# ICLDisco/parsec

Hardware: NVIDIA H100
Metric: tasks/s (higher is better)
Workload: dtype i32

## Files before the change

parsec_b200/csrc/pb2_stream.cu:

```cuda
#include <cuda_runtime.h>
#include <stdio.h>
#include <stdlib.h>
#include <string.h>
#include <atomic>
#include <deque>
#include <mutex>
#include <vector>

#include "../../include/pb2_stream.h"
#include "pb2_engine_priv.hpp"
#include "pb2_worker.cuh"

namespace pb2 {

enum : uint8_t { CMD_NONE = 0, CMD_TASK = 1, CMD_TILE = 2, CMD_EDGE = 3 };
enum : uint32_t { HS_STOPPED = 0, HS_RUNNING = 1, HS_ERROR = 2 };
constexpr int32_t kEdgeEmpty = -1;
constexpr int32_t kEdgeDone = -2;

struct alignas(64) Cmd {
    uint8_t  op, body, nb_flows, flags;
    uint16_t nparts, dep_goal;
    union {
        struct { int32_t ticket; int32_t tile[PB2_MAX_FLOWS]; uint8_t access[PB2_MAX_FLOWS];
                 int32_t iparam[3]; float fparam; int32_t locals[2]; } task;
        struct { int32_t tile; int32_t state; uint32_t version; int32_t src_kind;
                 uint64_t dev_ptr; uint64_t src_ptr; uint32_t bytes; } tset;
        struct { int32_t pred, succ, node; } edge;
        uint32_t raw[12];
    } u;
    uint32_t pad;
    uint32_t stamp;
};
static_assert(sizeof(Cmd) == 64, "Cmd must be one 64-byte line");

struct alignas(32) Retire {
    uint32_t seen[PB2_MAX_FLOWS];
    uint64_t result;
    int32_t  ticket;
    uint32_t stamp;
};
static_assert(sizeof(Retire) == 32, "Retire must be 32 bytes");

struct alignas(32) TraceRec { unsigned long long t_start, t_end; uint32_t smid; int32_t ticket; uint32_t pad[2]; };

struct HostCtl {
    volatile uint32_t state;
    volatile uint32_t stop_req;
    volatile uint32_t error;
    volatile uint32_t pad;
    char pad0[48];
    volatile unsigned long long cmd_consumed;
    char pad1[56];
};

struct SCtl {
    unsigned long long cmd_head;
    unsigned long long dispatched;
    Line published;
    Line released;
    Line edges_late;
};

struct StreamDev {
    WinDev w;
    const Cmd* cmd; uint32_t cmd_mask;
    Retire* ret;   uint32_t ret_mask;
    HostCtl* hctl;
    SCtl* sctl;
    int32_t* succ_head;
    int32_t* edge_next;
    int32_t* edge_succ;
    uint16_t* nparts_rw;
    pb2_task_t* tasks_rw;
    unsigned long long idle_ns;
    TraceRec* trace;
};

__device__ __forceinline__ uint32_t ld_volatile_u32(const volatile uint32_t* p) { return *p; }
__device__ __forceinline__ void st_volatile_v4(void* p, const uint4& v) {
    asm volatile("st.volatile.global.v4.u32 [%0], {%1,%2,%3,%4};" :: "l"(p), "r"(v.x), "r"(v.y), "r"(v.z), "r"(v.w) : "memory");
}
__device__ __forceinline__ void st_volatile_v2(void* p, uint32_t a, uint32_t b) {
    asm volatile("st.volatile.global.v2.u32 [%0], {%1,%2};" :: "l"(p), "r"(a), "r"(b) : "memory");
}

__device__ __forceinline__ void push_ready(const WinDev& w, int32_t slot, int np) {
    const uint32_t first = (uint32_t)atomicAdd(&w.ctl->tail.v, (unsigned long long)np);
    for (int p = 0; p < np; ++p) st_release_gpu(&w.ring[(first + (uint32_t)p) & w.cap_mask], PB2_ENT_MAKE(slot, p));
}

__device__ __forceinline__ int32_t stream_pop(const WinDev& w) {
    const uint32_t ticket = (uint32_t)atomicAdd(&w.ctl->head.v, 1ull);
    int32_t* slot = &w.ring[ticket & w.cap_mask];
    uint32_t spins = 0;
    int32_t id;
    while ((id = ld_acquire_gpu(slot)) == kEmpty) {
        if (ld_relaxed_gpu(reinterpret_cast<const int32_t*>(&w.ctl->done.v)) != 0) return kEmpty;
        ++spins;
        __nanosleep(spins < 64 ? 32 : 256);
    }
    st_relaxed_gpu(slot, kEmpty);
    return id;
}

__device__ __forceinline__ void dispatcher_warp(const StreamDev& sd) {
    const WinDev& w = sd.w;
    const int lane = threadIdx.x & 31;
    unsigned long long head = sd.sctl->cmd_head;
    unsigned long long dispatched = sd.sctl->dispatched;
    unsigned long long last_work = globaltimer_ns();
    if (lane == 0) { sd.hctl->state = HS_RUNNING; __threadfence_system(); }
    for (;;) {
        const unsigned long long idx = head + (unsigned long long)lane;
        const Cmd* c = &sd.cmd[idx & sd.cmd_mask];
        const uint32_t want = (uint32_t)(idx / ((unsigned long long)sd.cmd_mask + 1ull)) + 1u;
        const uint32_t got = ld_volatile_u32(&c->stamp);
        const unsigned validm = __ballot_sync(0xffffffffu, got == want);
        const int n = (validm == 0xffffffffu) ? 32 : (__ffs(~validm) - 1);
        if (n == 0) {
            int leave = 0;
            if (lane == 0) {
                const unsigned long long now = globaltimer_ns();
                const unsigned long long pub = *reinterpret_cast<volatile unsigned long long*>(&sd.sctl->published.v);
                const bool quiet = (pub == dispatched);
                if (quiet && (ld_volatile_u32(&sd.hctl->stop_req) != 0 || (long long)(now - last_work) > (long long)sd.idle_ns)) {
                    sd.hctl->state = HS_STOPPED;
                    __threadfence_system();
                    if (ld_volatile_u32(&sd.cmd[head & sd.cmd_mask].stamp) == (uint32_t)(head / ((unsigned long long)sd.cmd_mask + 1ull)) + 1u) {
                        sd.hctl->state = HS_RUNNING;
                        __threadfence_system();
                    } else leave = 1;
                } else if (!quiet) {
                    const unsigned long long last = *reinterpret_cast<volatile unsigned long long*>(&w.ctl->progress_ns.v);
                    const unsigned long long ref = last > last_work ? last : last_work;
                    if ((long long)(now - ref) > (long long)w.timeout_ns) {
                        sd.hctl->error = (uint32_t)kDoneTimeout; sd.hctl->state = HS_ERROR;
                        __threadfence_system();
                        st_relaxed_gpu(reinterpret_cast<int32_t*>(&w.ctl->done.v), kDoneTimeout);
                        leave = 2;
                    }
                } else if (ld_relaxed_gpu(reinterpret_cast<const int32_t*>(&w.ctl->done.v)) == kDoneBadBody) {
                    sd.hctl->error = (uint32_t)kDoneBadBody; sd.hctl->state = HS_ERROR;
                    __threadfence_system();
                    leave = 2;
                }
            }
            leave = __shfl_sync(0xffffffffu, leave, 0);
            if (leave) {
                if (lane == 0) {
                    sd.sctl->cmd_head = head; sd.sctl->dispatched = dispatched;
                    __threadfence();
                    if (leave == 1) st_release_gpu(reinterpret_cast<int32_t*>(&w.ctl->done.v), kDoneOK);
                }
                return;
            }
            __nanosleep(200);
            continue;
        }
        __threadfence_system();
        uint4 q0 = make_uint4(0, 0, 0, 0), q1 = q0, q2 = q0, q3 = q0;
        if (lane < n) {
            const uint4* p = reinterpret_cast<const uint4*>(c);
            q0 = ld_remote(p); q1 = ld_remote(p + 1); q2 = ld_remote(p + 2); q3 = ld_remote(p + 3);
        }
        const uint8_t op = (lane < n) ? (uint8_t)(q0.x & 0xffu) : (uint8_t)CMD_NONE;
        const int np = (int)(q0.y & 0xffffu), goal = (int)(q0.y >> 16);
        int32_t ticket = -1;
        if (op == CMD_TILE) {
            const int32_t tile = (int32_t)q0.z;
            if (tile >= 0 && tile < w.ntiles) {
                pb2_tile_t t;
                t.state = (int32_t)q0.w; t.version = q1.x; t.src_kind = (int32_t)q1.y;
                t.dev_ptr = reinterpret_cast<void*>(((unsigned long long)q1.w << 32) | q1.z);
                t.src_ptr = reinterpret_cast<void*>(((unsigned long long)q2.y << 32) | q2.x);
                t.bytes = q2.z;
                w.tiles[tile] = t;
                if (w.slice_claim && t.state != PB2_TILE_VALID) {
                    for (int k = 0; k < PB2_SLICE_WORDS; ++k) w.slice_claim[(size_t)tile * PB2_SLICE_WORDS + k] = 0;
                    for (int k = 0; k <= PB2_SLICE_WORDS; ++k) w.slice_done[(size_t)tile * (PB2_SLICE_WORDS + 1) + k] = 0;
                }
            }
        } else if (op == CMD_TASK) {
            ticket = (int32_t)q0.z;
            pb2_task_t t;
            t.dep_goal = goal; t.succ_begin = 0; t.succ_count = 0; t.priority = 0;
            t.body = (uint8_t)((q0.x >> 8) & 0xffu); t.nb_flows = (uint8_t)((q0.x >> 16) & 0xffu);
            t.flags = (uint8_t)(q0.x >> 24); t.class_id = 0;
            t.tile[0] = (int32_t)q0.w; t.tile[1] = (int32_t)q1.x; t.tile[2] = (int32_t)q1.y; t.tile[3] = (int32_t)q1.z;
            t.access[0] = (uint8_t)(q1.w & 0xffu); t.access[1] = (uint8_t)((q1.w >> 8) & 0xffu);
            t.access[2] = (uint8_t)((q1.w >> 16) & 0xffu); t.access[3] = (uint8_t)(q1.w >> 24);
            t.iparam[0] = (int32_t)q2.x; t.iparam[1] = (int32_t)q2.y; t.iparam[2] = (int32_t)q2.z;
            t.fparam = __uint_as_float(q2.w);
            t.locals[0] = (int32_t)q3.x; t.locals[1] = (int32_t)q3.y;
            sd.tasks_rw[ticket] = t;
            w.dep[ticket] = goal;
            sd.succ_head[ticket] = kEdgeEmpty;
            sd.nparts_rw[ticket] = (uint16_t)np;
            w.parts_left[ticket] = np;
            w.result[ticket] = 0;
        }
        __threadfence();
        __syncwarp();
        {
            const int mine = (op == CMD_TASK && goal == 0) ? np : 0;
            int incl = mine;
            for (int o = 1; o < 32; o <<= 1) { const int v = __shfl_up_sync(0xffffffffu, incl, o); if (lane >= o) incl += v; }
            const int total = __shfl_sync(0xffffffffu, incl, 31);
            if (total) {
                unsigned long long base = 0;
                if (lane == 0) base = atomicAdd(&w.ctl->tail.v, (unsigned long long)total);
                base = __shfl_sync(0xffffffffu, base, 0);
                push_entries_warp<false>(w.ring, w.cap_mask, ticket, mine, (uint32_t)base + (uint32_t)(incl - mine));
            }
        }
        if (op == CMD_EDGE) {
            const int32_t pred = (int32_t)q0.z, succ = (int32_t)q0.w, node = (int32_t)q1.x;
            sd.edge_succ[node] = succ;
            int32_t old = ld_acquire_gpu(&sd.succ_head[pred]);
            for (;;) {
                if (old == kEdgeDone) {
                    atomicAdd(&sd.sctl->edges_late.v, 1ull);
                    if (atomicSub(&w.dep[succ], 1) == 1) push_ready(w, succ, (int)sd.nparts_rw[succ]);
                    break;
                }
                sd.edge_next[node] = old;
                __threadfence();
                const int32_t seen = atomicCAS(&sd.succ_head[pred], old, node);
                if (seen == old) break;
                old = seen;
            }
        }
        const unsigned ntask = __popc(__ballot_sync(0xffffffffu, op == CMD_TASK));
        dispatched += ntask;
        head += (unsigned long long)n;
        last_work = globaltimer_ns();
        if (lane == 0) sd.hctl->cmd_consumed = head;
    }
}

#ifndef PB2_STREAM_MINB
#define PB2_STREAM_MINB 12
#endif
__global__ void __launch_bounds__(64, PB2_STREAM_MINB)
pb2_stream_kernel(StreamDev sd) {
    const WinDev& w = sd.w;
    if (blockIdx.x == 0) {
        if (threadIdx.x < 32) dispatcher_warp(sd);
        return;
    }
    __shared__ TaskSmem s;
    __shared__ BulkSmem bulk;
    if (threadIdx.x == 0) bulk_init(bulk);
    __syncthreads();
    for (;;) {
        if (threadIdx.x == 0) {
            const int32_t e = stream_pop(w);
            if (e != kEmpty) __threadfence();
            s.entry = e;
        }
        __syncthreads();
        const int32_t entry = s.entry;
        if (entry == kEmpty) break;
        const unsigned long long t_pop = (sd.trace != nullptr && threadIdx.x == 0) ? globaltimer_ns() : 0ull;
        const int32_t id = PB2_ENT_TASK(entry);
        const int part = PB2_ENT_PART(entry);
        if (threadIdx.x < 4) reinterpret_cast<uint4*>(&s.task)[threadIdx.x] =
            __ldcg(reinterpret_cast<const uint4*>(&w.tasks[id]) + threadIdx.x);
        __syncthreads();
        const int nparts = (int)__ldcg(&w.nparts[id]);
        const unsigned long long r = run_task_part<true>(w, s, &bulk, id, part, nparts,
                                                         [&] { return run_hbm_body(s.task.body, s.args, s.red); });

        if (threadIdx.x == 0) {
            __threadfence();
            const pb2_task_t& t = s.task;
            store_result(w, t, id, part, nparts, r);
            int last = 1;
            if (nparts > 1) { last = atomicSub(&w.parts_left[id], 1) == 1; __threadfence(); }
            if (last) {
                epilog_written_flows(w, t);
                const unsigned long long ridx = atomicAdd(&w.ctl->retired.v, 1ull);
                *reinterpret_cast<volatile unsigned long long*>(&w.ctl->progress_ns.v) = globaltimer_ns();
                __threadfence();
                int32_t node = atomicExch(&sd.succ_head[id], kEdgeDone);
                while (node >= 0) {
                    const int32_t succ = __ldcg(&sd.edge_succ[node]);
                    const int32_t next = __ldcg(&sd.edge_next[node]);
                    if (atomicSub(&w.dep[succ], 1) == 1) {
                        push_ready(w, succ, (int)__ldcg(&w.nparts[succ]));
                        atomicAdd(&sd.sctl->released.v, 1ull);
                    }
                    node = next;
                }
                if (sd.trace != nullptr) {
                    TraceRec* tr = &sd.trace[ridx & sd.ret_mask];
                    tr->t_start = t_pop; tr->t_end = globaltimer_ns(); tr->smid = smid(); tr->ticket = id;
                }
                Retire* rec = &sd.ret[ridx & sd.ret_mask];
                const uint32_t gen = (uint32_t)(ridx / ((unsigned long long)sd.ret_mask + 1ull)) + 1u;
                const uint4 lo = __ldcg(reinterpret_cast<const uint4*>(&w.seen_version[(size_t)id * PB2_MAX_FLOWS]));
                const unsigned long long res = *reinterpret_cast<volatile unsigned long long*>(&w.result[id]);
                uint4 hi;
                hi.x = (uint32_t)res; hi.y = (uint32_t)(res >> 32); hi.z = (uint32_t)id;
                hi.w = (gen & 0x7fffffffu) | (r == ~0ull ? 0x80000000u : 0u);
                bool host_reads = sd.trace != nullptr;
                for (int f = 0; f < (int)t.nb_flows; ++f) host_reads |= (t.access[f] & PB2_FLOW_PUSHOUT) != 0;
                if (host_reads) __threadfence_system();
                st_volatile_v4(rec, lo);
                st_volatile_v2(&rec->result, hi.x, hi.y);
                *reinterpret_cast<volatile int32_t*>(&rec->ticket) = (int32_t)hi.z;
                st_release_sys(reinterpret_cast<int32_t*>(&rec->stamp), (int32_t)hi.w);
                __threadfence_system();
                atomicAdd(&sd.sctl->published.v, 1ull);
            }
        }
        __syncthreads();
    }
}

__global__ void pb2_stream_rearm_kernel(StreamDev sd) {
    sd.w.ctl->head.v = 0; sd.w.ctl->tail.v = 0; sd.w.ctl->done.v = 0;
    sd.w.ctl->progress_ns.v = globaltimer_ns();
}

}

using namespace pb2;

struct DryTask { pb2_task_t t; int32_t dep; std::vector<int32_t> succ; bool done; };

struct pb2_stream_s {
    pb2_engine_t* e = nullptr;
    pb2_stream_params_t p{};
    bool dry = false;
    std::string last_error;
    uint32_t slots = 0, ring_cap = 0;
    Cmd* h_cmd = nullptr; Retire* h_ret = nullptr; HostCtl* h_ctl = nullptr; TraceRec* h_trace = nullptr;
    StreamDev d{};
    std::vector<void*> dev_allocs;
    cudaStream_t kstream = nullptr;
    int nworkers = 0;
    unsigned long long cmd_written = 0;
    unsigned long long consumed_seen = 0;
    std::vector<int32_t> free_tickets, free_nodes;
    std::vector<uint64_t> cookie;
    std::vector<uint16_t> tk_parts;
    std::vector<std::vector<int32_t>> tk_nodes;
    std::vector<uint8_t> tk_live;
    alignas(64) unsigned long long ret_read = 0;
    std::vector<int32_t> freed;
    alignas(64) std::atomic<uint64_t> freed_tail{0};
    alignas(64) std::atomic<uint64_t> freed_head{0};
    alignas(64) std::atomic<uint64_t> sub_tasks{0};
    std::atomic<uint64_t> sub_entries{0};
    uint64_t ret_entries_seen = 0;
    alignas(64) std::atomic<uint64_t> ret_tasks{0};
    std::atomic<uint64_t> ret_entries{0};
    std::mutex launch_mu;
    std::mutex nodes_mu;
    std::mutex dry_mu;
    pb2_stream_stats_t st{};
    std::vector<DryTask> dry_tasks;
    std::deque<int32_t> dry_ready;
    std::vector<pb2_tile_t> dry_tiles;
    std::vector<uint32_t> tile_bytes;
};

#define STREAM_CUDA(s, call)                                                                     \
    do {                                                                                         \
        cudaError_t err__ = (call);                                                              \
        if (err__ != cudaSuccess) {                                                              \
            char buf__[512];                                                                     \
            snprintf(buf__, sizeof buf__, "%s:%d %s -> %s", __FILE__, __LINE__, #call,           \
                     cudaGetErrorString(err__));                                                 \
            (s)->last_error = buf__;                                                             \
            fprintf(stderr, "pb2: CUDA error %s\n", buf__);                                      \
            return PB2_ERR_DEVICE;                                                               \
        }                                                                                        \
    } while (0)

template <class T>
static int sdev_alloc(pb2_stream_t* s, T** out, size_t n, int fill) {
    void* ptr = nullptr;
    STREAM_CUDA(s, cudaMalloc(&ptr, (n ? n : 1) * sizeof(T)));
    STREAM_CUDA(s, cudaMemset(ptr, fill, (n ? n : 1) * sizeof(T)));
    s->dev_allocs.push_back(ptr);
    *out = reinterpret_cast<T*>(ptr);
    return PB2_SUCCESS;
}

static uint32_t round_pow2(uint32_t v, uint32_t lo, uint32_t hi) {
    uint32_t r = lo;
    while (r < v && r < hi) r <<= 1;
    return r;
}

extern "C" {

const char* pb2_stream_last_error(pb2_stream_t* s) { return s ? s->last_error.c_str() : "null stream"; }

int pb2_stream_create(pb2_engine_t* e, const pb2_stream_params_t* params, pb2_stream_t** stream) {
    if (!stream) return PB2_ERR_BAD_PARAM;
    *stream = nullptr;
    pb2_stream_params_t p{};
    if (params) p = *params;
    if (!e && !p.dry_run) return PB2_ERR_BAD_PARAM;
    if (p.cmd_slots <= 0) p.cmd_slots = 65536;
    if (p.max_tiles <= 0) p.max_tiles = 65536;
    if (p.idle_us <= 0) p.idle_us = 2000;
    if (p.timeout_ms <= 0) p.timeout_ms = 20000;
    if (p.part_bytes == 0) p.part_bytes = kDefaultPartBytes;
    pb2_stream_t* s = new pb2_stream_s();
    s->e = e; s->p = p; s->dry = p.dry_run != 0;
    s->slots = round_pow2((uint32_t)p.cmd_slots, 1024u, 1u << 21);
    s->ring_cap = s->slots * 4u;
    s->free_tickets.reserve(s->slots); s->free_nodes.reserve(s->slots);
    for (int32_t i = (int32_t)s->slots - 1; i >= 0; --i) { s->free_tickets.push_back(i); s->free_nodes.push_back(i); }
    s->tile_bytes.assign((size_t)p.max_tiles, 0);
    s->cookie.assign(s->slots, 0); s->tk_parts.assign(s->slots, 1); s->tk_nodes.resize(s->slots); s->tk_live.assign(s->slots, 0);
    s->freed.assign(s->slots, -1);
    if (s->dry) {
        s->dry_tasks.resize(s->slots);
        s->dry_tiles.resize((size_t)p.max_tiles);
        *stream = s;
        return PB2_SUCCESS;
    }
    STREAM_CUDA(s, cudaSetDevice(e->cuda_device));
    STREAM_CUDA(s, cudaHostAlloc(reinterpret_cast<void**>(&s->h_cmd), sizeof(Cmd) * s->slots, cudaHostAllocMapped | cudaHostAllocPortable));
    STREAM_CUDA(s, cudaHostAlloc(reinterpret_cast<void**>(&s->h_ret), sizeof(Retire) * s->slots, cudaHostAllocMapped | cudaHostAllocPortable));
    STREAM_CUDA(s, cudaHostAlloc(reinterpret_cast<void**>(&s->h_ctl), sizeof(HostCtl), cudaHostAllocMapped | cudaHostAllocPortable));
    memset(s->h_cmd, 0, sizeof(Cmd) * s->slots);
    memset(s->h_ret, 0, sizeof(Retire) * s->slots);
    memset((void*)s->h_ctl, 0, sizeof(HostCtl));
    StreamDev& d = s->d;
    void* alias = nullptr;
    STREAM_CUDA(s, cudaHostGetDevicePointer(&alias, s->h_cmd, 0)); d.cmd = reinterpret_cast<const Cmd*>(alias);
    STREAM_CUDA(s, cudaHostGetDevicePointer(&alias, s->h_ret, 0)); d.ret = reinterpret_cast<Retire*>(alias);
    STREAM_CUDA(s, cudaHostGetDevicePointer(&alias, (void*)s->h_ctl, 0)); d.hctl = reinterpret_cast<HostCtl*>(alias);
    d.cmd_mask = s->slots - 1; d.ret_mask = s->slots - 1;
    if (p.trace) {
        STREAM_CUDA(s, cudaHostAlloc(reinterpret_cast<void**>(&s->h_trace), sizeof(TraceRec) * s->slots, cudaHostAllocMapped | cudaHostAllocPortable));
        memset(s->h_trace, 0, sizeof(TraceRec) * s->slots);
        STREAM_CUDA(s, cudaHostGetDevicePointer(&alias, s->h_trace, 0)); d.trace = reinterpret_cast<TraceRec*>(alias);
    }
    int rc;
#define TRY(x) do { rc = (x); if (rc != PB2_SUCCESS) { pb2_stream_destroy(s); return rc; } } while (0)
    WinDev& w = d.w;
    memset(&w, 0, sizeof w);
    TRY(sdev_alloc(s, &d.tasks_rw, s->slots, 0)); w.tasks = d.tasks_rw;
    TRY(sdev_alloc(s, &w.tiles, (size_t)p.max_tiles, 0));
    TRY(sdev_alloc(s, &w.dep, s->slots, 0));
    TRY(sdev_alloc(s, &w.ring, s->ring_cap, 0xff));
    TRY(sdev_alloc(s, &w.ctl, 1, 0));
    TRY(sdev_alloc(s, &w.seen_version, (size_t)s->slots * PB2_MAX_FLOWS, 0));
    TRY(sdev_alloc(s, &w.result, s->slots, 0));
    TRY(sdev_alloc(s, &w.parts_left, s->slots, 0));
    TRY(sdev_alloc(s, &d.nparts_rw, s->slots, 0)); w.nparts = d.nparts_rw;
    TRY(sdev_alloc(s, &w.slice_claim, (size_t)p.max_tiles * PB2_SLICE_WORDS, 0));
    TRY(sdev_alloc(s, &w.slice_done, (size_t)p.max_tiles * (PB2_SLICE_WORDS + 1), 0));
    TRY(sdev_alloc(s, &d.sctl, 1, 0));
    TRY(sdev_alloc(s, &d.succ_head, s->slots, 0xff));
    TRY(sdev_alloc(s, &d.edge_next, s->slots, 0xff));
    TRY(sdev_alloc(s, &d.edge_succ, s->slots, 0xff));
#undef TRY
    w.cap_mask = s->ring_cap - 1; w.ntasks = (int32_t)s->slots; w.ntiles = p.max_tiles;
    w.stage_mode = e->params.stage_mode;
    w.part_bytes = stage_slice(e->stage_slice_bytes, p.part_bytes);
    w.timeout_ns = (unsigned long long)p.timeout_ms * 1000000ull;
    d.idle_ns = (unsigned long long)p.idle_us * 1000ull;
    STREAM_CUDA(s, cudaStreamCreateWithFlags(&s->kstream, cudaStreamNonBlocking));
    int occ = 0;
    STREAM_CUDA(s, cudaOccupancyMaxActiveBlocksPerMultiprocessor(&occ, pb2_stream_kernel, 64, 0));
    if (occ > PB2_STREAM_MINB) occ = PB2_STREAM_MINB;
    if (occ < 1) occ = 1;
    s->nworkers = e->prop.multiProcessorCount * occ;
    if (p.max_workers > 0 && p.max_workers + 1 < s->nworkers) s->nworkers = p.max_workers + 1;
    if (s->nworkers < 2) s->nworkers = 2;
    *stream = s;
    return PB2_SUCCESS;
}

int pb2_stream_destroy(pb2_stream_t* s) {
    if (!s) return PB2_ERR_BAD_PARAM;
    if (!s->dry) {
        cudaSetDevice(s->e->cuda_device);
        if (s->kstream) {
            if (s->h_ctl) s->h_ctl->stop_req = 1;
            cudaStreamSynchronize(s->kstream);
            cudaStreamDestroy(s->kstream);
        }
        for (void* p : s->dev_allocs) cudaFree(p);
        if (s->h_cmd) cudaFreeHost(s->h_cmd);
        if (s->h_ret) cudaFreeHost(s->h_ret);
        if (s->h_ctl) cudaFreeHost((void*)s->h_ctl);
        if (s->h_trace) cudaFreeHost(s->h_trace);
    }
    delete s;
    return PB2_SUCCESS;
}

static int stream_launch_if_parked(pb2_stream_t* s) {
    if (s->dry) return PB2_SUCCESS;
    std::atomic_thread_fence(std::memory_order_seq_cst);
    uint32_t st = s->h_ctl->state;
    if (st == HS_RUNNING) return PB2_SUCCESS;
    if (st == HS_ERROR) { s->last_error = "streaming kernel aborted (watchdog or unknown body)"; return PB2_ERR_DEVICE; }
    std::lock_guard<std::mutex> guard(s->launch_mu);
    st = s->h_ctl->state;
    if (st == HS_RUNNING) return PB2_SUCCESS;
    if (st == HS_ERROR) { s->last_error = "streaming kernel aborted (watchdog or unknown body)"; return PB2_ERR_DEVICE; }
    STREAM_CUDA(s, cudaSetDevice(s->e->cuda_device));
    s->h_ctl->state = HS_RUNNING;
    std::atomic_thread_fence(std::memory_order_seq_cst);
    pb2_stream_rearm_kernel<<<1, 1, 0, s->kstream>>>(s->d);
    pb2_stream_kernel<<<s->nworkers, 64, 0, s->kstream>>>(s->d);
    STREAM_CUDA(s, cudaGetLastError());
    s->st.kernel_launches++;
    return PB2_SUCCESS;
}

static int stream_cmd_slot(pb2_stream_t* s, Cmd** out) {
    if (s->cmd_written - s->consumed_seen >= (unsigned long long)s->slots) s->consumed_seen = s->h_ctl->cmd_consumed;
    if (s->cmd_written - s->consumed_seen >= (unsigned long long)s->slots) {
        int rc = stream_launch_if_parked(s);
        if (rc != PB2_SUCCESS) return rc;
        unsigned long long spins = 0;
        while (s->cmd_written - s->h_ctl->cmd_consumed >= (unsigned long long)s->slots) {
            if (s->h_ctl->state == HS_ERROR) { s->last_error = "streaming kernel aborted"; return PB2_ERR_DEVICE; }
            if ((++spins & 0xfffff) == 0 && s->h_ctl->state == HS_STOPPED) { rc = stream_launch_if_parked(s); if (rc != PB2_SUCCESS) return rc; }
        }
        s->consumed_seen = s->h_ctl->cmd_consumed;
    }
    *out = &s->h_cmd[s->cmd_written & (s->slots - 1)];
    __builtin_prefetch(&s->h_cmd[(s->cmd_written + 6) & (s->slots - 1)], 1, 3);
    return PB2_SUCCESS;
}
static void stream_cmd_publish(pb2_stream_t* s, Cmd* c) {
    const uint32_t gen = (uint32_t)(s->cmd_written / (unsigned long long)s->slots) + 1u;
    std::atomic_thread_fence(std::memory_order_release);
    *reinterpret_cast<volatile uint32_t*>(&c->stamp) = gen;
    s->cmd_written++;
}

int pb2_stream_set_tile(pb2_stream_t* s, int32_t tile, const pb2_tile_t* desc) {
    if (!s || !desc || tile < 0 || tile >= s->p.max_tiles) return PB2_ERR_BAD_PARAM;
    s->tile_bytes[(size_t)tile] = desc->bytes;
    if (s->dry) { s->dry_tiles[(size_t)tile] = *desc; return PB2_SUCCESS; }
    Cmd* c;
    int rc = stream_cmd_slot(s, &c);
    if (rc != PB2_SUCCESS) return rc;
    memset(c, 0, 60);
    c->op = CMD_TILE;
    c->u.tset.tile = tile; c->u.tset.state = desc->state; c->u.tset.version = desc->version; c->u.tset.src_kind = desc->src_kind;
    c->u.tset.dev_ptr = (uint64_t)(uintptr_t)desc->dev_ptr; c->u.tset.src_ptr = (uint64_t)(uintptr_t)desc->src_ptr;
    c->u.tset.bytes = desc->bytes;
    stream_cmd_publish(s, c);
    return PB2_SUCCESS;
}

int pb2_stream_submit(pb2_stream_t* s, const pb2_task_t* task, uint64_t cookie, int32_t* ticket) {
    if (!s || !task) return PB2_ERR_BAD_PARAM;
    if (task->nb_flows > PB2_MAX_FLOWS) { s->last_error = "task with more than PB2_MAX_FLOWS flows"; return PB2_ERR_BAD_PARAM; }
    if (task->body >= PB2_BODY_MAX || task->body == PB2_BODY_USER || task->body == PB2_BODY_GEMM_BF16) {
        s->last_error = "body cannot run in the streaming kernel"; return PB2_ERR_NOT_SUPPORTED; }
    if (task->dep_goal < 0 || task->dep_goal > 0xffff) return PB2_ERR_VALUE_OUT_OF_BOUNDS;
    for (int f = 0; f < task->nb_flows; ++f)
        if (task->tile[f] >= s->p.max_tiles) { s->last_error = "tile id out of bounds"; return PB2_ERR_VALUE_OUT_OF_BOUNDS; }
    if (s->free_tickets.empty()) {
        uint64_t h = s->freed_head.load(std::memory_order_relaxed);
        const uint64_t t = s->freed_tail.load(std::memory_order_acquire);
        for (; h != t; ++h) s->free_tickets.push_back(s->freed[h & (s->slots - 1)]);
        s->freed_head.store(h, std::memory_order_release);
        if (s->free_tickets.empty()) return PB2_ERR_OUT_OF_RESOURCE;
    }
    const uint32_t np = (uint32_t)task_parts(*task, [&](int32_t id) { return s->tile_bytes[(size_t)id]; },
                                             s->p.part_bytes, PB2_MAX_PARTS);
    {
        const uint64_t sub = s->sub_entries.load(std::memory_order_relaxed);
        if (sub - s->ret_entries_seen + np + 64 > (uint64_t)s->ring_cap / 2) {
            s->ret_entries_seen = s->ret_entries.load(std::memory_order_acquire);
            if (sub - s->ret_entries_seen + np + 64 > (uint64_t)s->ring_cap / 2) return PB2_ERR_OUT_OF_RESOURCE;
        }
    }
    const int32_t tk = s->free_tickets.back();
    if (s->dry) {
        std::lock_guard<std::mutex> guard(s->dry_mu);
        s->free_tickets.pop_back();
        s->cookie[(size_t)tk] = cookie; s->tk_parts[(size_t)tk] = (uint16_t)np; s->tk_live[(size_t)tk] = 1;
        s->sub_entries.store(s->sub_entries.load(std::memory_order_relaxed) + np, std::memory_order_relaxed);
        s->sub_tasks.store(s->sub_tasks.load(std::memory_order_relaxed) + 1, std::memory_order_release);
        if (ticket) *ticket = tk;
        DryTask& dt = s->dry_tasks[(size_t)tk];
        dt.t = *task; dt.dep = task->dep_goal; dt.succ.clear(); dt.done = false;
        if (dt.dep == 0) s->dry_ready.push_back(tk);
    } else {
        Cmd* c;
        int rc = stream_cmd_slot(s, &c);
        if (rc != PB2_SUCCESS) return rc;
        s->free_tickets.pop_back();
        s->cookie[(size_t)tk] = cookie; s->tk_parts[(size_t)tk] = (uint16_t)np; s->tk_live[(size_t)tk] = 1;
        memset(c, 0, 60);
        c->op = CMD_TASK; c->body = task->body; c->nb_flows = task->nb_flows; c->flags = task->flags;
        c->nparts = (uint16_t)np; c->dep_goal = (uint16_t)task->dep_goal;
        c->u.task.ticket = tk;
        for (int f = 0; f < PB2_MAX_FLOWS; ++f) { c->u.task.tile[f] = f < task->nb_flows ? task->tile[f] : -1; c->u.task.access[f] = task->access[f]; }
        c->u.task.iparam[0] = task->iparam[0]; c->u.task.iparam[1] = task->iparam[1]; c->u.task.iparam[2] = task->iparam[2];
        c->u.task.fparam = task->fparam; c->u.task.locals[0] = task->locals[0]; c->u.task.locals[1] = task->locals[1];
        s->sub_entries.store(s->sub_entries.load(std::memory_order_relaxed) + np, std::memory_order_relaxed);
        s->sub_tasks.store(s->sub_tasks.load(std::memory_order_relaxed) + 1, std::memory_order_release);
        if (ticket) *ticket = tk;
        stream_cmd_publish(s, c);
    }
    return PB2_SUCCESS;
}

int pb2_stream_add_edge(pb2_stream_t* s, int32_t pred, int32_t succ) {
    if (!s || pred < 0 || succ < 0 || pred >= (int32_t)s->slots || succ >= (int32_t)s->slots) return PB2_ERR_BAD_PARAM;
    if (!s->tk_live[(size_t)pred] || !s->tk_live[(size_t)succ]) { s->last_error = "edge names a ticket that is not in flight"; return PB2_ERR_BAD_PARAM; }
    s->st.edges++;
    if (s->dry) {
        std::lock_guard<std::mutex> guard(s->dry_mu);
        DryTask& p = s->dry_tasks[(size_t)pred];
        if (p.done) { if (--s->dry_tasks[(size_t)succ].dep == 0) s->dry_ready.push_back(succ); }
        else p.succ.push_back(succ);
        return PB2_SUCCESS;
    }
    Cmd* c;
    int rc = stream_cmd_slot(s, &c);
    if (rc != PB2_SUCCESS) return rc;
    int32_t node;
    {
        std::lock_guard<std::mutex> guard(s->nodes_mu);
        if (s->free_nodes.empty()) return PB2_ERR_OUT_OF_RESOURCE;
        node = s->free_nodes.back(); s->free_nodes.pop_back();
        s->tk_nodes[(size_t)pred].push_back(node);
    }
    memset(c, 0, 60);
    c->op = CMD_EDGE; c->u.edge.pred = pred; c->u.edge.succ = succ; c->u.edge.node = node;
    stream_cmd_publish(s, c);
    return PB2_SUCCESS;
}

int pb2_stream_kick(pb2_stream_t* s) {
    if (!s) return PB2_ERR_BAD_PARAM;
    if (s->dry || s->cmd_written == 0) return PB2_SUCCESS;
    return stream_launch_if_parked(s);
}

int pb2_stream_poll(pb2_stream_t* s, pb2_retire_t* out, int32_t max) {
    if (!s || (max > 0 && !out)) return PB2_ERR_BAD_PARAM;
    int n = 0;
    if (s->dry) {
        std::lock_guard<std::mutex> guard(s->dry_mu);
        while (n < max && !s->dry_ready.empty()) {
            const int32_t tk = s->dry_ready.front(); s->dry_ready.pop_front();
            DryTask& dt = s->dry_tasks[(size_t)tk];
            dt.done = true;
            pb2_retire_t& r = out[n++];
            memset(&r, 0, sizeof r);
            r.cookie = s->cookie[(size_t)tk]; r.ticket = tk; r.status = PB2_SUCCESS;
            for (int f = 0; f < dt.t.nb_flows && f < PB2_MAX_FLOWS; ++f) {
                if (dt.t.tile[f] < 0) continue;
                pb2_tile_t& tl = s->dry_tiles[(size_t)dt.t.tile[f]];
                r.seen_version[f] = tl.version;
                if (dt.t.access[f] & PB2_FLOW_ACCESS_WRITE) tl.version++;
                tl.state = PB2_TILE_VALID;
            }
            for (int32_t sc : dt.succ) if (--s->dry_tasks[(size_t)sc].dep == 0) s->dry_ready.push_back(sc);
            dt.succ.clear();
            s->tk_live[(size_t)tk] = 0;
            const uint64_t ft = s->freed_tail.load(std::memory_order_relaxed);
            s->freed[ft & (s->slots - 1)] = tk;
            s->freed_tail.store(ft + 1, std::memory_order_release);
            s->ret_entries.store(s->ret_entries.load(std::memory_order_relaxed) + s->tk_parts[(size_t)tk], std::memory_order_release);
            s->ret_tasks.store(s->ret_tasks.load(std::memory_order_relaxed) + 1, std::memory_order_release);
        }
        return n;
    }
    if (s->h_ctl->state == HS_ERROR) {
        s->last_error = s->h_ctl->error == (uint32_t)kDoneTimeout ? "streaming kernel watchdog: no task retired within timeout"
                                                                  : "streaming kernel ran a task with an unknown body id";
        return s->h_ctl->error == (uint32_t)kDoneTimeout ? PB2_ERR_DEVICE : PB2_ERR_BAD_PARAM;
    }
    if (s->h_ctl->state == HS_STOPPED && s->sub_tasks.load(std::memory_order_acquire) != s->ret_tasks.load(std::memory_order_relaxed)) {
        const Retire* nxt = &s->h_ret[s->ret_read & (s->slots - 1)];
        const uint32_t g = ((uint32_t)(s->ret_read / (unsigned long long)s->slots) + 1u) & 0x7fffffffu;
        if ((*reinterpret_cast<const volatile uint32_t*>(&nxt->stamp) & 0x7fffffffu) != g) {
            int rc = stream_launch_if_parked(s);
            if (rc != PB2_SUCCESS) return rc;
        }
    }
    while (n < max) {
        const Retire* rec = &s->h_ret[s->ret_read & (s->slots - 1)];
        __builtin_prefetch(&s->h_ret[(s->ret_read + 8) & (s->slots - 1)], 0, 3);
        const uint32_t gen = ((uint32_t)(s->ret_read / (unsigned long long)s->slots) + 1u) & 0x7fffffffu;
        const uint32_t stamp = *reinterpret_cast<const volatile uint32_t*>(&rec->stamp);
        if ((stamp & 0x7fffffffu) != gen) break;
        std::atomic_thread_fence(std::memory_order_acquire);
        const int32_t tk = *reinterpret_cast<const volatile int32_t*>(&rec->ticket);
        pb2_retire_t& r = out[n++];
        r.cookie = s->cookie[(size_t)tk]; r.result = *reinterpret_cast<const volatile uint64_t*>(&rec->result);
        for (int f = 0; f < PB2_MAX_FLOWS; ++f) r.seen_version[f] = *reinterpret_cast<const volatile uint32_t*>(&rec->seen[f]);
        r.ticket = tk; r.status = (stamp & 0x80000000u) ? PB2_ERR_BAD_PARAM : PB2_SUCCESS;
        if (s->h_trace) {
            const volatile TraceRec* tr = &s->h_trace[s->ret_read & (s->slots - 1)];
            r.t_start_ns = tr->t_start; r.t_end_ns = tr->t_end; r.smid = tr->smid; r.pad = 0;
        } else { r.t_start_ns = 0; r.t_end_ns = 0; r.smid = 0; r.pad = 0; }
        if (!s->tk_nodes[(size_t)tk].empty()) {
            std::lock_guard<std::mutex> guard(s->nodes_mu);
            for (int32_t nd : s->tk_nodes[(size_t)tk]) s->free_nodes.push_back(nd);
            s->tk_nodes[(size_t)tk].clear();
        }
        s->tk_live[(size_t)tk] = 0;
        const uint64_t ft = s->freed_tail.load(std::memory_order_relaxed);
        s->freed[ft & (s->slots - 1)] = tk;
        s->freed_tail.store(ft + 1, std::memory_order_release);
        s->ret_entries.store(s->ret_entries.load(std::memory_order_relaxed) + s->tk_parts[(size_t)tk], std::memory_order_release);
        s->ret_tasks.store(s->ret_tasks.load(std::memory_order_relaxed) + 1, std::memory_order_release);
        s->ret_read++;
    }
    return n;
}

int pb2_stream_quiesce(pb2_stream_t* s) {
    if (!s) return PB2_ERR_BAD_PARAM;
    if (s->dry) return PB2_SUCCESS;
    STREAM_CUDA(s, cudaSetDevice(s->e->cuda_device));
    if (s->cmd_written != s->h_ctl->cmd_consumed) { int rc = stream_launch_if_parked(s); if (rc != PB2_SUCCESS) return rc; }
    s->h_ctl->stop_req = 1;
    std::atomic_thread_fence(std::memory_order_seq_cst);
    STREAM_CUDA(s, cudaStreamSynchronize(s->kstream));
    s->h_ctl->stop_req = 0;
    if (s->h_ctl->state == HS_ERROR) { s->last_error = "streaming kernel aborted"; return PB2_ERR_DEVICE; }
    if (s->cmd_written != s->h_ctl->cmd_consumed) return pb2_stream_quiesce(s);
    return PB2_SUCCESS;
}

int pb2_stream_inflight(pb2_stream_t* s) { return s ? (int)(s->sub_tasks.load() - s->ret_tasks.load()) : 0; }

int pb2_stream_stats(pb2_stream_t* s, pb2_stream_stats_t* out) {
    if (!s || !out) return PB2_ERR_BAD_PARAM;
    if (!s->dry) {
        STREAM_CUDA(s, cudaSetDevice(s->e->cuda_device));
        Ctl c; SCtl sc;
        cudaStream_t aux = s->e->up_stream;
        STREAM_CUDA(s, cudaMemcpyAsync(&c, s->d.w.ctl, sizeof c, cudaMemcpyDeviceToHost, aux));
        STREAM_CUDA(s, cudaMemcpyAsync(&sc, s->d.sctl, sizeof sc, cudaMemcpyDeviceToHost, aux));
        STREAM_CUDA(s, cudaStreamSynchronize(aux));
        s->st.bytes_h2d = c.bytes_h2d.v; s->st.bytes_d2d = c.bytes_d2d.v; s->st.bytes_d2h = c.bytes_d2h.v;
        s->st.stage_ins = c.stage_ins.v; s->st.body_errors = c.body_errors.v;
        s->st.edges_late = sc.edges_late.v; s->st.released_on_device = sc.released.v;
    }
    s->st.submitted = s->sub_tasks.load(); s->st.retired = s->ret_tasks.load();
    *out = s->st;
    return PB2_SUCCESS;
}

}
```

parsec_b200/mca/b200/device_b200_module.c:

```c
#include "parsec/parsec_config.h"
#include "parsec/parsec_internal.h"
#include "parsec/sys/atomic.h"
#include "parsec/utils/mca_param.h"
#include "parsec/utils/debug.h"
#include "parsec/utils/zone_malloc.h"
#include "parsec/constants.h"
#include "parsec/data_internal.h"
#include "parsec/scheduling.h"
#include "parsec/execution_stream.h"
#include "parsec/mca/device/device.h"
#include "parsec/mca/device/device_gpu.h"
#include "parsec/mca/device/b200/device_b200.h"
#include "parsec/mca/device/b200/device_b200_internal.h"

#include "pb2_engine.h"
#include "pb2_stream.h"

#include <cuda_runtime_api.h>
#include <stddef.h>
#include <stdlib.h>
#include <string.h>
#include <stdio.h>
#include <limits.h>
#include <time.h>
static inline uint64_t b200_now_ns(void) { struct timespec ts; clock_gettime(CLOCK_MONOTONIC, &ts); return (uint64_t)ts.tv_sec * 1000000000ull + (uint64_t)ts.tv_nsec; }
#include <x86intrin.h>
#define B200_TSC() __rdtsc()

#include <nvtx3/nvToolsExt.h>
static nvtxDomainHandle_t b200_nvtx_domain = NULL;
static inline void b200_nvtx_attr(nvtxEventAttributes_t *a, const char *name)
{
    memset(a, 0, sizeof *a);
    a->version = NVTX_VERSION; a->size = NVTX_EVENT_ATTRIB_STRUCT_SIZE;
    a->messageType = NVTX_MESSAGE_TYPE_ASCII; a->message.ascii = name;
}
static inline void b200_nvtx_push(const char *name)
{
    if( parsec_b200_nvtx ) { nvtxEventAttributes_t a; b200_nvtx_attr(&a, name); (void)nvtxDomainRangePushEx(b200_nvtx_domain, &a); }
}
static inline void b200_nvtx_pop(void)
{
    if( parsec_b200_nvtx ) (void)nvtxDomainRangePop(b200_nvtx_domain);
}
static inline void b200_nvtx_mark(const char *name)
{
    if( parsec_b200_nvtx ) { nvtxEventAttributes_t a; b200_nvtx_attr(&a, name); nvtxDomainMarkEx(b200_nvtx_domain, &a); }
}

typedef struct b200_lock_s {
    volatile uint32_t next;    char pad0[60];
    volatile uint32_t serving; char pad1[60];
} b200_lock_t;
static inline void b200_lock(b200_lock_t *l)
{
    const uint32_t t = __atomic_fetch_add(&l->next, 1, __ATOMIC_RELAXED);
    while( __atomic_load_n(&l->serving, __ATOMIC_ACQUIRE) != t ) _mm_pause();
}
static inline void b200_unlock(b200_lock_t *l)
{
    __atomic_store_n(&l->serving, l->serving + 1, __ATOMIC_RELEASE);
}

enum {
    BT_NEW = 0,
    BT_STAGED,
    BT_DMA_IN,
    BT_INFLIGHT,
    BT_LANE,
    BT_DMA_OUT
};

typedef struct b200_task_s {
    parsec_list_item_t   item;
    parsec_gpu_task_t   *gpu_task;
    int32_t              state;
    int32_t              ticket;
    int32_t              body;
    int32_t              prepared;
    int32_t              cmd_built;
    int32_t              recorded;
    int32_t              has_complete_stage;
    uint32_t             dma_out_mask;
    uint64_t             result;
    uint64_t             cold_bytes;
    struct parsec_device_b200_module_s *dev;
    int32_t              is_kernel;
    int32_t              defer_tiles;
    int32_t              ntdesc;
    pb2_task_t           cmd __attribute__((aligned(64)));
    parsec_task_t        proxy __attribute__((aligned(64)));
    int32_t              nb_args;
    int32_t              arg_flow[PB2_MAX_FLOWS];
    int32_t              iparam[3];
    float                fparam;
    uint32_t             peer_src_mask;
    parsec_data_copy_t  *peer_src[MAX_PARAM_COUNT];
    int32_t              custom_stage;
    cudaEvent_t          ev;
    int32_t              ev_dev;
    struct b200_task_s  *next_free;
    struct b200_task_s  *next_done;
    struct { int32_t tile; pb2_tile_t desc; } tdesc[MAX_PARAM_COUNT];
} b200_task_t;

typedef struct b200_host_range_s { char *base; size_t len; char *alias; int lazy; } b200_host_range_t;

typedef struct b200_trace_ev_s {
    char     name[24];
    int32_t  locals[2];
    int32_t  body, smid;
    uint64_t t_start_ns, t_end_ns, cold_bytes;
} b200_trace_ev_t;
#define B200_LINE __attribute__((aligned(64)))
typedef struct parsec_device_b200_module_s {
    parsec_device_cuda_module_t super;
    pb2_engine_t        *engine;
    pb2_stream_t        *stream;
    int                  dry_run;
    char                *slab_base;
    uint8_t             *tile_described;
    b200_task_t * volatile *inbox_ring;
    cudaStream_t         dma_stream;
    parsec_cuda_exec_stream_t *lane;
    uint64_t             first_entry_ns, first_task_ns, last_done_ns;
    volatile int64_t     inbox_tail B200_LINE;
    volatile int32_t     owed B200_LINE;
    volatile int32_t     callers_inside B200_LINE;
    volatile int32_t     max_callers_inside;
    volatile int64_t     epilogs_done B200_LINE;
    b200_lock_t          lru_lock B200_LINE;
    b200_lock_t          alloc_lock B200_LINE;
    volatile int32_t     handed_back B200_LINE;
    volatile int32_t     starter_active B200_LINE;
    volatile int32_t     fatal;
    volatile int32_t     memory_pressure;
    struct b200_task_s * volatile lane_done;
    volatile int32_t     retry_stalled B200_LINE;
    volatile int64_t     cold_inflight B200_LINE;
    volatile int64_t     inbox_head B200_LINE;
    parsec_list_t        stalled B200_LINE;
    parsec_list_t        settled;
    parsec_list_t        cold_q;
    int32_t              nb_cold;
    parsec_list_t        waiting_event;
    int32_t              nb_settled;
    int32_t              nb_stalled;
    int32_t              again_window;
    int32_t              lane_pending;
    uint64_t             n_engine, n_lane, n_settled_by_caller;
    uint64_t             tsc_start[4];
    uint64_t             tsc_s[3];
    parsec_list_t        waiting_out B200_LINE;
    parsec_task_t       *completion_ring;
    b200_task_t         *batch_head;
    int32_t              batch_len;
    int32_t              completed_now;
    int32_t              blocked_spins;
    int32_t              complete_inline;
    int64_t              epilogs_started;
    uint64_t             tsc[8];
    struct b200_trace_ev_s *trace_ev;
    size_t               trace_n, trace_cap;
    pb2_retire_t         retbuf[256];
    parsec_b200_stats_t  st B200_LINE;
} parsec_device_b200_module_t;

static b200_host_range_t *b200_ranges = NULL;
static int b200_nb_ranges = 0, b200_cap_ranges = 0;
static parsec_atomic_lock_t b200_ranges_lock = PARSEC_ATOMIC_UNLOCKED;

static int  parsec_b200_submit_is_engine(parsec_advance_task_function_t fn);
static void parsec_b200_submit_set_engine(parsec_advance_task_function_t fn);

#define B200_DEV(gpu)   ((parsec_device_b200_module_t*)(gpu))
#define B200_BT(gt)     ((b200_task_t*)(uintptr_t)(gt)->last_data_check_epoch)

#define B200_CUDA(call, what, onerr)                                                              \
    do { cudaError_t e__ = (call); if( cudaSuccess != e__ ) {                                     \
        parsec_warning("device_b200: %s: %s", (what), cudaGetErrorString(e__)); onerr; } } while(0)

int parsec_b200_is_b200_device(const parsec_device_module_t *device)
{
    return (NULL != device) && (device->component == &parsec_device_b200_component);
}

int parsec_b200_device_count(void)
{
    int n = 0;
    if( cudaSuccess != cudaGetDeviceCount(&n) ) { (void)cudaGetLastError(); return 0; }
    return n;
}

static char *b200_device_visible(const void *host_ptr, size_t len)
{
    char *res = NULL;
    parsec_atomic_lock(&b200_ranges_lock);
    for( int i = 0; i < b200_nb_ranges; i++ ) {
        const b200_host_range_t *r = &b200_ranges[i];
        if( (const char*)host_ptr >= r->base && (const char*)host_ptr + len <= r->base + r->len ) {
            res = r->alias + ((const char*)host_ptr - r->base);
            break;
        }
    }
    parsec_atomic_unlock(&b200_ranges_lock);
    return res;
}

#define B200_INBOX_SLOTS (1 << 16)
#define B200_TL_CACHE    8192
#define B200_FLAG_WRITER ((parsec_data_flag_t)1 << 4)
static __thread b200_task_t *b200_tl_free = NULL;
static __thread int          b200_tl_nfree = 0;
static __thread b200_task_t *b200_tl_recording = NULL;

static parsec_hook_return_t b200_epilog_hook(parsec_execution_stream_t *es, parsec_task_t *task);
static const __parsec_chore_t b200_completion_chores[] = {
    { .type = PARSEC_DEV_CPU, .evaluate = NULL, .hook = b200_epilog_hook, .dyld = NULL, .dyld_fn = NULL },
    { .type = PARSEC_DEV_NONE, .evaluate = NULL, .hook = NULL, .dyld = NULL, .dyld_fn = NULL },
};
static const parsec_task_class_t b200_completion_tc = {
    .name = "b200 completion", .flags = 0, .task_class_id = 0, .nb_flows = 0, .nb_parameters = 0, .nb_locals = 0,
    .incarnations = b200_completion_chores,
};

static b200_task_t *b200_bt_new(parsec_device_b200_module_t *dev, parsec_gpu_task_t *gpu_task)
{
    b200_task_t *bt = b200_tl_free;
    if( NULL != bt ) { b200_tl_free = bt->next_free; b200_tl_nfree--; }
    else {
        if( 0 != posix_memalign((void**)&bt, 64, sizeof(b200_task_t)) ) abort();
        memset(bt, 0, sizeof(b200_task_t));
        PARSEC_OBJ_CONSTRUCT(&bt->item, parsec_list_item_t);
        PARSEC_OBJ_CONSTRUCT(&bt->proxy, parsec_task_t);
        bt->proxy.task_class = &b200_completion_tc;
        bt->proxy.priority = INT32_MAX;
        bt->proxy.status = PARSEC_TASK_STATUS_HOOK;
        bt->proxy.chore_mask = 1;
        bt->proxy.selected_chore = 0;
        bt->proxy.selected_device = parsec_mca_device_get(0);
        bt->proxy.load = 0;
        bt->proxy.repo_entry = NULL;
        bt->ev_dev = -1;
    }
    PARSEC_LIST_ITEM_SINGLETON(&bt->item);
    bt->dev = dev;
    bt->gpu_task = gpu_task; bt->state = BT_NEW; bt->ticket = -1; bt->body = -1; bt->nb_args = 0;
    bt->peer_src_mask = 0; bt->dma_out_mask = 0; bt->result = 0; bt->custom_stage = 0; bt->cold_bytes = 0;
    bt->recorded = 0; bt->has_complete_stage = 0; bt->prepared = 0; bt->cmd_built = 0; bt->defer_tiles = 0; bt->ntdesc = 0;
    bt->is_kernel = (NULL == gpu_task) || (PARSEC_GPU_TASK_TYPE_KERNEL == gpu_task->task_type);
    if( NULL != gpu_task ) gpu_task->last_data_check_epoch = (uint64_t)(uintptr_t)bt;
    return bt;
}

static void b200_bt_free(b200_task_t *bt)
{
    bt->gpu_task = NULL;
    if( b200_tl_nfree < B200_TL_CACHE ) { bt->next_free = b200_tl_free; b200_tl_free = bt; b200_tl_nfree++; return; }
    if( bt->ev_dev >= 0 ) (void)cudaEventDestroy(bt->ev);
    free(bt);
}

static inline void b200_cuda_here(parsec_device_b200_module_t *dev)
{
    if( !dev->dry_run ) B200_CUDA(cudaSetDevice(dev->super.cuda_index), "cudaSetDevice", {});
}

static cudaEvent_t b200_bt_event(parsec_device_b200_module_t *dev, b200_task_t *bt)
{
    if( bt->ev_dev != (int32_t)dev->super.cuda_index ) {
        if( bt->ev_dev >= 0 ) (void)cudaEventDestroy(bt->ev);
        bt->ev_dev = -1;
        b200_cuda_here(dev);
        B200_CUDA(cudaEventCreateWithFlags(&bt->ev, cudaEventDisableTiming), "cudaEventCreate", { return bt->ev; });
        bt->ev_dev = (int32_t)dev->super.cuda_index;
    }
    return bt->ev;
}

static inline void b200_lru_put(parsec_device_b200_module_t *dev, parsec_list_t *list, parsec_data_copy_t *copy)
{
    b200_lock(&dev->lru_lock);
    copy->flags &= (parsec_data_flag_t)~B200_FLAG_WRITER;
    parsec_list_item_ring_chop((parsec_list_item_t*)copy); PARSEC_LIST_ITEM_SINGLETON(copy);
    parsec_list_nolock_push_back(list, (parsec_list_item_t*)copy);
    b200_unlock(&dev->lru_lock);
}
static inline void b200_lru_take(parsec_device_b200_module_t *dev, parsec_data_copy_t *copy, int for_writer)
{
    b200_lock(&dev->lru_lock);
    if( for_writer ) copy->flags |= B200_FLAG_WRITER;
    parsec_list_item_ring_chop((parsec_list_item_t*)copy); PARSEC_LIST_ITEM_SINGLETON(copy);
    b200_unlock(&dev->lru_lock);
}
static inline void b200_lru_touch(parsec_device_b200_module_t *dev, parsec_data_copy_t *copy)
{
    b200_lock(&dev->lru_lock);
    if( !(copy->flags & B200_FLAG_WRITER) ) {
        parsec_list_t *l = (PARSEC_DATA_COHERENCY_OWNED == copy->coherency_state) ? &dev->super.super.gpu_mem_owned_lru
                                                                                  : &dev->super.super.gpu_mem_lru;
        parsec_list_item_ring_chop((parsec_list_item_t*)copy); PARSEC_LIST_ITEM_SINGLETON(copy);
        parsec_list_nolock_push_back(l, (parsec_list_item_t*)copy);
    }
    b200_unlock(&dev->lru_lock);
}

#define B200_PF(p) __builtin_prefetch((const void*)(p), 0, 3)
#define B200_PFW(p) __builtin_prefetch((const void*)(p), 1, 3)
static inline void b200_pf1(const b200_task_t *bt)
{
    const char *g = (const char*)bt->gpu_task;
    if( NULL != g ) { B200_PF(g); B200_PF(g + 64); B200_PF(g + 128); }
}
static inline void b200_pf2(const b200_task_t *bt)
{
    const parsec_gpu_task_t *g = bt->gpu_task;
    if( NULL == g || NULL == g->ec ) return;
    const parsec_task_t *t = g->ec;
    B200_PF(t); B200_PF((const char*)t + 64);
    B200_PF(&t->data[0]); B200_PF((const char*)&t->data[0] + 64);
    B200_PF(g->flow_info);
}
static inline void b200_pf3(const b200_task_t *bt)
{
    const parsec_gpu_task_t *g = bt->gpu_task;
    if( NULL == g || NULL == g->ec ) return;
    const uint32_t n = g->nb_flows < 4 ? g->nb_flows : 4;
    for( uint32_t i = 0; i < n; i++ ) {
        if( NULL != g->ec->data[i].data_in ) B200_PF(g->ec->data[i].data_in);
        if( NULL != g->ec->data[i].data_out ) B200_PF(g->ec->data[i].data_out);
    }
}
static inline void b200_pf4(const b200_task_t *bt)
{
    const parsec_gpu_task_t *g = bt->gpu_task;
    if( NULL == g || NULL == g->ec ) return;
    const uint32_t n = g->nb_flows < 4 ? g->nb_flows : 4;
    for( uint32_t i = 0; i < n; i++ ) {
        const parsec_data_copy_t *c = (NULL != g->ec->data[i].data_in) ? g->ec->data[i].data_in : g->ec->data[i].data_out;
        if( NULL != c && NULL != c->original ) { B200_PF(c->original); B200_PF((const char*)c->original + 64); }
    }
}

static inline int32_t b200_tile_of(const parsec_device_b200_module_t *dev, const parsec_data_copy_t *gpu_copy)
{
    return (int32_t)(((char*)gpu_copy->device_private - dev->slab_base) / (ptrdiff_t)dev->super.super.mem_block_size);
}

static int b200_copy_acquire_reader(parsec_data_copy_t *copy)
{
    int32_t r = copy->readers;
    while( r >= 0 ) {
        if( parsec_atomic_cas_int32(&copy->readers, r, r + 1) ) return 1;
        r = copy->readers;
    }
    return 0;
}

static void b200_release_copy_memory(parsec_device_b200_module_t *dev, parsec_data_copy_t *copy)
{
    parsec_data_t *original = copy->original;
    if( NULL != original ) {
        parsec_atomic_lock(&original->lock);
        const int survives = original->super.obj_reference_count != 1;
        parsec_data_copy_detach(original, copy, dev->super.super.super.device_index);
        parsec_atomic_wmb();
        if( survives ) parsec_atomic_unlock(&original->lock);
    }
    if( NULL != dev->tile_described ) dev->tile_described[b200_tile_of(dev, copy)] = 0;
    zone_free(dev->super.super.memory, copy->device_private);
    copy->device_private = NULL;
    PARSEC_OBJ_RELEASE(copy);
    dev->super.super.super.nb_evictions++;
    dev->st.evictions++;
}

static int b200_write_back_some(parsec_device_b200_module_t *dev, int how_many)
{
    parsec_list_item_t *it, *next;
    parsec_data_copy_t *moved[64];
    int done = 0;
    if( how_many > 64 ) how_many = 64;
    b200_lock(&dev->lru_lock);
    for( it = PARSEC_LIST_ITERATOR_FIRST(&dev->super.super.gpu_mem_owned_lru);
         it != PARSEC_LIST_ITERATOR_END(&dev->super.super.gpu_mem_owned_lru) && done < how_many; it = next ) {
        parsec_data_copy_t *copy = (parsec_data_copy_t*)it;
        next = PARSEC_LIST_ITERATOR_NEXT(it);
        if( 0 != copy->readers || (copy->flags & B200_FLAG_WRITER) ) continue;
        parsec_data_copy_t *cpu = copy->original->device_copies[0];
        if( NULL == cpu || (!dev->dry_run && NULL == cpu->device_private) ) continue;
        parsec_list_nolock_remove(&dev->super.super.gpu_mem_owned_lru, it);
        PARSEC_LIST_ITEM_SINGLETON(it);
        moved[done++] = copy;
    }
    b200_unlock(&dev->lru_lock);
    if( 0 == done ) return 0;
    if( !dev->dry_run ) {
        b200_cuda_here(dev);
        for( int i = 0; i < done; i++ ) {
            parsec_data_copy_t *copy = moved[i], *cpu = copy->original->device_copies[0];
            B200_CUDA(cudaMemcpyAsync(cpu->device_private, copy->device_private, copy->original->span, cudaMemcpyDeviceToHost, dev->dma_stream),
                      "write-back cudaMemcpyAsync", { moved[i] = NULL; b200_lru_put(dev, &dev->super.super.gpu_mem_owned_lru, copy); continue; });
            (void)parsec_atomic_fetch_add_int64((volatile int64_t*)&dev->super.super.super.data_out_to_host, (int64_t)copy->original->span);
            dev->st.bytes_d2h_dma += copy->original->span;
        }
        B200_CUDA(cudaStreamSynchronize(dev->dma_stream), "write-back synchronize", {});
    }
    int n = 0;
    for( int i = 0; i < done; i++ ) {
        parsec_data_copy_t *copy = moved[i];
        if( NULL == copy ) continue;
        parsec_data_copy_t *cpu = copy->original->device_copies[0];
        parsec_atomic_lock(&copy->original->lock);
        if( cpu->version < copy->version ) cpu->version = copy->version;
        cpu->coherency_state = PARSEC_DATA_COHERENCY_SHARED;
        copy->coherency_state = PARSEC_DATA_COHERENCY_SHARED;
        if( copy->original->owner_device == (int8_t)dev->super.super.super.device_index ) copy->original->owner_device = 0;
        parsec_atomic_unlock(&copy->original->lock);
        b200_lru_put(dev, &dev->super.super.gpu_mem_lru, copy);
        dev->st.w2r_copies++;
        n++;
    }
    return n;
}

static int b200_evict_one(parsec_device_b200_module_t *dev, const parsec_gpu_task_t *for_task)
{
    for( int pass = 0; pass < 2; pass++ ) {
        parsec_list_item_t *it, *next;
        parsec_data_copy_t *victim = NULL;
        b200_lock(&dev->lru_lock);
        for( it = PARSEC_LIST_ITERATOR_FIRST(&dev->super.super.gpu_mem_lru);
             it != PARSEC_LIST_ITERATOR_END(&dev->super.super.gpu_mem_lru); it = next ) {
            parsec_data_copy_t *copy = (parsec_data_copy_t*)it;
            next = PARSEC_LIST_ITERATOR_NEXT(it);
            if( PARSEC_DATA_STATUS_UNDER_TRANSFER == copy->data_transfer_status || (copy->flags & B200_FLAG_WRITER) ) continue;
            if( copy->super.super.obj_reference_count > 1 ) continue;
            if( NULL != for_task ) {
                int mine = 0;
                for( uint32_t f = 0; f < for_task->nb_flows; f++ )
                    mine |= (for_task->ec->data[f].data_out == copy) || (for_task->ec->data[f].data_in == copy);
                if( mine ) continue;
            }
            if( !parsec_atomic_cas_int32(&copy->readers, 0, INT_MIN / 2) ) continue;
            parsec_data_copy_t *cpu = (NULL != copy->original) ? copy->original->device_copies[0] : NULL;
            if( NULL != copy->original && (NULL == cpu || cpu->version < copy->version) &&
                copy->original->owner_device == (int8_t)dev->super.super.super.device_index ) {
                copy->readers = 0;
                continue;
            }
            parsec_list_nolock_remove(&dev->super.super.gpu_mem_lru, it);
            PARSEC_LIST_ITEM_SINGLETON(it);
            victim = copy;
            break;
        }
        b200_unlock(&dev->lru_lock);
        if( NULL != victim ) {
            victim->readers = 0;
            b200_release_copy_memory(dev, victim);
            return 1;
        }
        if( 0 == b200_write_back_some(dev, 16) ) break;
    }
    return 0;
}

static int b200_reserve(parsec_device_b200_module_t *dev, b200_task_t *bt)
{
    parsec_gpu_task_t *gpu_task = bt->gpu_task;
    parsec_task_t *this_task = gpu_task->ec;
    const uint8_t my = dev->super.super.super.device_index;
    parsec_data_copy_t *fresh[MAX_PARAM_COUNT];
    int nfresh = 0;

    for( uint32_t i = 0; i < gpu_task->nb_flows; i++ ) {
        const parsec_flow_t *flow = gpu_task->flow_info[i].flow;
        if( PARSEC_FLOW_ACCESS_NONE == (PARSEC_FLOW_ACCESS_MASK & flow->flow_flags) ) { gpu_task->flow_info[i].flow_span = 0; continue; }
        parsec_data_copy_t *in = this_task->data[i].data_in;
        if( NULL == in ) continue;
        if( in->device_index == my ) { this_task->data[i].data_out = in; continue; }
        parsec_data_t *master = in->original;
        parsec_atomic_lock(&master->lock);
        parsec_data_copy_t *gpu_elem = PARSEC_DATA_GET_COPY(master, my);
        parsec_atomic_unlock(&master->lock);
        if( NULL == gpu_elem ) {
            void *ptr;
            while( NULL == (ptr = zone_malloc(dev->super.super.memory, gpu_task->flow_info[i].flow_span)) ) {
                dev->memory_pressure = 1;
                if( !b200_evict_one(dev, gpu_task) ) {
                    for( int k = 0; k < nfresh; k++ ) {
                        b200_lru_take(dev, fresh[k], 0);
                        b200_release_copy_memory(dev, fresh[k]);
                        dev->super.super.super.nb_evictions--; dev->st.evictions--;
                    }
                    for( uint32_t k = 0; k < gpu_task->nb_flows; k++ )
                        if( NULL != this_task->data[k].data_in && this_task->data[k].data_in->device_index != my ) this_task->data[k].data_out = NULL;
                    return PARSEC_HOOK_RETURN_AGAIN;
                }
            }
            gpu_elem = PARSEC_OBJ_NEW(parsec_data_copy_t);
            gpu_elem->flags = PARSEC_DATA_FLAG_PARSEC_OWNED | PARSEC_DATA_FLAG_PARSEC_MANAGED;
            gpu_elem->device_private = ptr;
            gpu_elem->arena_chunk = (parsec_arena_chunk_t*)dev->super.super.memory;
            gpu_elem->coherency_state = PARSEC_DATA_COHERENCY_INVALID;
            gpu_elem->version = 0;
            gpu_elem->dtt = in->dtt;
            parsec_atomic_lock(&master->lock);
            parsec_data_copy_attach(master, gpu_elem, my);
            parsec_atomic_unlock(&master->lock);
            b200_lru_put(dev, &dev->super.super.gpu_mem_lru, gpu_elem);
            fresh[nfresh++] = gpu_elem;
        }
        this_task->data[i].data_out = gpu_elem;
    }
    return PARSEC_HOOK_RETURN_DONE;
}

static int b200_needs_memory(const parsec_device_b200_module_t *dev, const parsec_gpu_task_t *gpu_task)
{
    const uint8_t my = dev->super.super.super.device_index;
    for( uint32_t i = 0; i < gpu_task->nb_flows; i++ ) {
        const parsec_flow_t *flow = gpu_task->flow_info[i].flow;
        if( PARSEC_FLOW_ACCESS_NONE == (PARSEC_FLOW_ACCESS_MASK & flow->flow_flags) ) continue;
        const parsec_data_copy_t *in = gpu_task->ec->data[i].data_in;
        if( NULL == in || in->device_index == my ) continue;
        if( NULL == PARSEC_DATA_GET_COPY(in->original, my) ) return 1;
    }
    return 0;
}

static int b200_emit_tile(parsec_device_b200_module_t *dev, b200_task_t *bt, int32_t tid, const pb2_tile_t *tile)
{
    if( !bt->defer_tiles ) return (PB2_SUCCESS == pb2_stream_set_tile(dev->stream, tid, tile)) ? 0 : -1;
    if( bt->ntdesc >= MAX_PARAM_COUNT ) return -1;
    bt->tdesc[bt->ntdesc].tile = tid; bt->tdesc[bt->ntdesc].desc = *tile; bt->ntdesc++;
    return 0;
}

static int b200_stage_in(parsec_device_b200_module_t *dev, b200_task_t *bt, int mode)
{
    const int for_lane = (0 != mode);
    parsec_gpu_task_t *gpu_task = bt->gpu_task;
    parsec_task_t *this_task = gpu_task->ec;
    parsec_device_module_t *mod = &dev->super.super.super;
    const uint8_t my = mod->device_index;
    int used_dma = 0;
    uint32_t pre_acquired = 0;

    for( uint32_t i = 0; i < gpu_task->nb_flows; i++ ) {
        const parsec_flow_t *flow = gpu_task->flow_info[i].flow;
        parsec_data_copy_t *in = this_task->data[i].data_in;
        if( NULL == in || NULL == this_task->data[i].data_out || in == this_task->data[i].data_out ) continue;
        if( !(PARSEC_FLOW_ACCESS_READ & flow->flow_flags) || !parsec_mca_device_is_gpu(in->device_index) ) continue;
        if( b200_copy_acquire_reader(in) ) { pre_acquired |= (1u << i); continue; }
        for( uint32_t k = 0; k < i; k++ )
            if( pre_acquired & (1u << k) ) (void)parsec_atomic_fetch_dec_int32(&this_task->data[k].data_in->readers);
        return PARSEC_HOOK_RETURN_AGAIN;
    }

    for( uint32_t i = 0; i < gpu_task->nb_flows; i++ ) {
        const parsec_flow_t *flow = gpu_task->flow_info[i].flow;
        const uint8_t type = (uint8_t)(flow->flow_flags & PARSEC_FLOW_ACCESS_MASK);
        if( PARSEC_FLOW_ACCESS_NONE == type ) continue;
        parsec_data_copy_t *in = this_task->data[i].data_in, *out = this_task->data[i].data_out;
        if( NULL == in || NULL == out ) continue;
        parsec_data_t *original = in->original;
        const size_t span = gpu_task->flow_info[i].flow_span;
        gpu_task->flow_info[i].source = NULL;

        if( in == out ) {
            if( PARSEC_FLOW_ACCESS_WRITE & type ) {
                out->version++;
                b200_lru_take(dev, out, 1);
                parsec_atomic_lock(&original->lock);
                original->owner_device = my; out->coherency_state = PARSEC_DATA_COHERENCY_OWNED;
                parsec_atomic_unlock(&original->lock);
            }
            if( PARSEC_FLOW_ACCESS_READ & type ) (void)parsec_atomic_fetch_inc_int32(&out->readers);
            if( !for_lane && !dev->tile_described[b200_tile_of(dev, out)] ) {
                pb2_tile_t tile;
                memset(&tile, 0, sizeof tile);
                tile.dev_ptr = out->device_private; tile.bytes = (uint32_t)span; tile.state = PB2_TILE_VALID;
                tile.version = (PARSEC_FLOW_ACCESS_WRITE & type) ? out->version - 1 : out->version;
                if( NULL != original->device_copies[0] && NULL != original->device_copies[0]->device_private )
                    tile.src_ptr = b200_device_visible(original->device_copies[0]->device_private, span);
                if( 0 != b200_emit_tile(dev, bt, b200_tile_of(dev, out), &tile) ) return PARSEC_HOOK_RETURN_ERROR;
                dev->tile_described[b200_tile_of(dev, out)] = 1;
            }
            continue;
        }

        parsec_atomic_lock(&original->lock);
        if( PARSEC_FLOW_ACCESS_WRITE & type ) {
            b200_lru_take(dev, out, 1);
        }
        parsec_data_copy_t *src = in;
        int src_acquired = 0, src_detour = 0;
        if( (PARSEC_FLOW_ACCESS_READ & type) ) {
            if( parsec_mca_device_is_gpu(in->device_index) ) {
                src_acquired = (pre_acquired >> i) & 1;
                src_detour = !(dev->super.super.peer_access_mask & (1 << in->device_index));
            } else if( !(PARSEC_FLOW_ACCESS_WRITE & type) ) {
                for( uint32_t t = 1; t < parsec_nb_devices; t++ ) {
                    parsec_data_copy_t *cand = original->device_copies[t];
                    if( t == my || NULL == cand || !(dev->super.super.peer_access_mask & (1 << t)) ) continue;
                    if( cand->version != in->version || PARSEC_DATA_COHERENCY_INVALID == cand->coherency_state ||
                        PARSEC_DATA_STATUS_UNDER_TRANSFER == cand->data_transfer_status ) continue;
                    if( b200_copy_acquire_reader(cand) ) { src = cand; src_acquired = 1; break; }
                }
            }
        }
        if( NULL == src ) { parsec_atomic_unlock(&original->lock); return PARSEC_HOOK_RETURN_ERROR; }

        int transfer_from = parsec_data_start_transfer_ownership_to_copy(original, my, type);
        if( -1 != transfer_from && out->version == src->version && PARSEC_DATA_STATUS_COMPLETE_TRANSFER == out->data_transfer_status ) transfer_from = -1;
        if( NULL == src->device_private ) transfer_from = -1;
        if( (NULL == this_task->data[i].source_repo_entry) && (NULL == original->dc) && (0 == in->version) ) transfer_from = -1;
        if( PARSEC_DATA_STATUS_UNDER_TRANSFER == out->data_transfer_status ) transfer_from = -1;
        mod->required_data_in += original->span;

        pb2_tile_t tile;
        memset(&tile, 0, sizeof tile);
        tile.dev_ptr = out->device_private;
        tile.bytes = (uint32_t)span;
        tile.state = PB2_TILE_VALID;
        tile.src_kind = parsec_mca_device_is_gpu(src->device_index) ? PB2_SRC_PEER : PB2_SRC_HOST;
        char *home = NULL;
        if( NULL != original->device_copies[0] && NULL != original->device_copies[0]->device_private )
            home = b200_device_visible(original->device_copies[0]->device_private, span);
        tile.src_ptr = home;

        if( -1 == transfer_from ) {
            if( src_acquired ) { (void)parsec_atomic_fetch_dec_int32(&src->readers); src_acquired = 0; }
            if( PARSEC_DATA_STATUS_UNDER_TRANSFER != out->data_transfer_status ) {
                out->data_transfer_status = PARSEC_DATA_STATUS_COMPLETE_TRANSFER;
                parsec_data_end_transfer_ownership_to_copy(original, my, type);
            }
            if( PARSEC_FLOW_ACCESS_WRITE & type ) out->version = src->version + 1;
        } else {
            char *visible = (PB2_SRC_PEER == tile.src_kind) ? (char*)src->device_private
                                                            : b200_device_visible(src->device_private, span);
            mod->data_in_from_device[src->device_index] += span;
            mod->nb_data_faults += span;
            bt->cold_bytes += span;
            if( PB2_SRC_PEER == tile.src_kind ) { if( src_detour ) dev->st.peer_detours++; else dev->st.peer_pulls++; }
            if( NULL != visible && !src_detour && !for_lane && !dev->dry_run ) {
                tile.state = PB2_TILE_INVALID;
                tile.src_ptr = visible;
                out->data_transfer_status = PARSEC_DATA_STATUS_UNDER_TRANSFER;
                if( PB2_SRC_PEER == tile.src_kind ) dev->st.bytes_d2d_kernel += span; else dev->st.bytes_h2d_kernel += span;
            } else if( 2 == mode ) {
                out->data_transfer_status = PARSEC_DATA_STATUS_UNDER_TRANSFER;
                used_dma = 1;
            } else if( !dev->dry_run ) {
                b200_cuda_here(dev);
                B200_CUDA(cudaMemcpyAsync(out->device_private, src->device_private, span,
                                          PB2_SRC_PEER == tile.src_kind ? cudaMemcpyDeviceToDevice : cudaMemcpyHostToDevice,
                                          for_lane ? dev->lane->cuda_stream : dev->dma_stream),
                          "stage-in cudaMemcpyAsync", { parsec_atomic_unlock(&original->lock); return PARSEC_HOOK_RETURN_ERROR; });
                out->data_transfer_status = PARSEC_DATA_STATUS_UNDER_TRANSFER;
                dev->st.bytes_h2d_dma += span;
                used_dma = 1;
            } else {
                out->data_transfer_status = PARSEC_DATA_STATUS_UNDER_TRANSFER;
            }
            out->version = (PARSEC_FLOW_ACCESS_WRITE & type) ? src->version + 1 : src->version;
            gpu_task->flow_info[i].source = src;
            if( src_acquired ) { bt->peer_src_mask |= (1u << i); bt->peer_src[i] = src; }
            if( PB2_SRC_PEER == tile.src_kind && PB2_TILE_INVALID == tile.state && NULL != home && (gpu_task->pushout & (1 << i)) ) {
            }
        }
        tile.version = (PARSEC_FLOW_ACCESS_WRITE & type) ? out->version - 1 : out->version;
        if( !for_lane ) {
            const int32_t tid = b200_tile_of(dev, out);
            if( -1 != transfer_from || !dev->tile_described[tid] ) {
                if( 0 != b200_emit_tile(dev, bt, tid, &tile) ) { parsec_atomic_unlock(&original->lock); return PARSEC_HOOK_RETURN_ERROR; }
                dev->tile_described[tid] = 1;
            }
        }
        parsec_atomic_unlock(&original->lock);
    }
    return used_dma;
}

int parsec_b200_task_body(parsec_device_gpu_module_t *gpu_device, parsec_gpu_task_t *gpu_task,
                          parsec_gpu_exec_stream_t *gpu_stream,
                          int body, int nb_args, const int *flow_index, const int32_t *iparam, float fparam)
{
    if( NULL == gpu_device || NULL == gpu_task || nb_args < 0 || nb_args > PB2_MAX_FLOWS || body < 0 || body >= PB2_BODY_MAX )
        return PARSEC_HOOK_RETURN_ERROR;
    for( int a = 0; a < nb_args; a++ )
        if( flow_index[a] < 0 || (uint32_t)flow_index[a] >= gpu_task->nb_flows ) return PARSEC_HOOK_RETURN_ERROR;
    if( parsec_b200_is_b200_device(&gpu_device->super) ) {
        b200_task_t *bt = b200_tl_recording;
        if( NULL == bt || bt->gpu_task != gpu_task ) return PARSEC_HOOK_RETURN_ERROR;
        bt->body = body; bt->nb_args = nb_args;
        for( int a = 0; a < nb_args; a++ ) bt->arg_flow[a] = flow_index[a];
        bt->iparam[0] = iparam ? iparam[0] : 0; bt->iparam[1] = iparam ? iparam[1] : 0; bt->iparam[2] = iparam ? iparam[2] : 0;
        bt->fparam = fparam;
        return PARSEC_HOOK_RETURN_DONE;
    }
    {
        void *ptrs[PB2_MAX_FLOWS] = {NULL, NULL, NULL, NULL};
        uint64_t bytes[PB2_MAX_FLOWS] = {0, 0, 0, 0};
        int32_t ip[3] = { iparam ? iparam[0] : 0, iparam ? iparam[1] : 0, iparam ? iparam[2] : 0 };
        for( int a = 0; a < nb_args; a++ ) {
            ptrs[a] = gpu_task->ec->data[flow_index[a]].data_out->device_private;
            bytes[a] = gpu_task->flow_info[flow_index[a]].flow_span;
        }
        parsec_cuda_exec_stream_t *cs = (parsec_cuda_exec_stream_t*)gpu_stream;
        return (PB2_SUCCESS == pb2_body_launch((void*)cs->cuda_stream, body, nb_args, ptrs, bytes, ip, fparam))
               ? PARSEC_HOOK_RETURN_DONE : PARSEC_HOOK_RETURN_ERROR;
    }
}

uint64_t parsec_b200_task_result(const parsec_gpu_task_t *gpu_task)
{
    const b200_task_t *bt = (const b200_task_t*)(uintptr_t)gpu_task->last_data_check_epoch;
    return (NULL != bt) ? bt->result : 0;
}

static inline void b200_stat_add(uint64_t *counter, uint64_t v)
{
    (void)parsec_atomic_fetch_add_int64((volatile int64_t*)counter, (int64_t)v);
}

static int b200_epilog_flows(parsec_device_b200_module_t *dev, b200_task_t *bt, parsec_data_copy_t **held)
{
    parsec_gpu_task_t *gpu_task = bt->gpu_task;
    parsec_task_t *this_task = gpu_task->ec;
    parsec_device_module_t *mod = &dev->super.super.super;
    int nheld = 0;

    for( uint32_t i = 0; i < gpu_task->nb_flows; i++ ) {
        const parsec_flow_t *flow = gpu_task->flow_info[i].flow;
        const uint8_t type = (uint8_t)(flow->flow_flags & PARSEC_FLOW_ACCESS_MASK);
        if( PARSEC_FLOW_ACCESS_NONE == type || NULL == this_task->data[i].data_in ) continue;
        parsec_data_copy_t *gpu_copy = this_task->data[i].data_out;
        if( NULL == gpu_copy ) continue;
        parsec_data_t *original = gpu_copy->original;
        const int locked = (PARSEC_FLOW_ACCESS_WRITE & type) || PARSEC_DATA_STATUS_UNDER_TRANSFER == gpu_copy->data_transfer_status;
        if( locked ) parsec_atomic_lock(&original->lock);
        if( PARSEC_DATA_STATUS_UNDER_TRANSFER == gpu_copy->data_transfer_status ) {
            gpu_copy->data_transfer_status = PARSEC_DATA_STATUS_COMPLETE_TRANSFER;
            parsec_data_end_transfer_ownership_to_copy(original, mod->device_index, type);
        }
        if( bt->peer_src_mask & (1u << i) ) (void)parsec_atomic_fetch_dec_int32(&bt->peer_src[i]->readers);
        if( !(PARSEC_FLOW_ACCESS_READ & type) ) (void)parsec_atomic_fetch_inc_int32(&gpu_copy->readers);
        held[nheld++] = gpu_copy;
        if( PARSEC_FLOW_ACCESS_WRITE & type ) {
            b200_stat_add(&mod->required_data_out, gpu_task->flow_info[i].flow_span);
            if( gpu_task->pushout & (1 << i) ) {
                parsec_data_copy_t *cpu_copy = original->device_copies[0];
                if( NULL != cpu_copy ) {
                    cpu_copy->version = gpu_copy->version;
                    cpu_copy->coherency_state = PARSEC_DATA_COHERENCY_SHARED;
                    gpu_copy->coherency_state = PARSEC_DATA_COHERENCY_SHARED;
                    cpu_copy->data_transfer_status = PARSEC_DATA_STATUS_COMPLETE_TRANSFER;
                    b200_stat_add(&mod->data_out_to_host, gpu_task->flow_info[i].flow_span);
                    if( 0 == (parsec_mpi_allow_gpu_memory_communications & PARSEC_RUNTIME_SEND_GPU_MEMORY) )
                        this_task->data[i].data_out = cpu_copy;
                }
                b200_lru_put(dev, &dev->super.super.gpu_mem_lru, gpu_copy);
            } else {
                gpu_copy->coherency_state = PARSEC_DATA_COHERENCY_OWNED;
                b200_lru_put(dev, &dev->super.super.gpu_mem_owned_lru, gpu_copy);
            }
        } else if( dev->memory_pressure && 1 == gpu_copy->readers && 0 != (gpu_copy->flags & PARSEC_DATA_FLAG_PARSEC_OWNED) ) {
            b200_lru_touch(dev, gpu_copy);
        }
        if( locked ) parsec_atomic_unlock(&original->lock);
    }
    return nheld;
}

static parsec_hook_return_t b200_epilog_hook(parsec_execution_stream_t *es, parsec_task_t *task)
{
    b200_task_t *bt = (b200_task_t*)((char*)task - offsetof(b200_task_t, proxy));
    parsec_device_b200_module_t *dev = bt->dev;
    int64_t n = 0;
    b200_nvtx_push("b200 epilog batch");
    while( NULL != bt ) {
        b200_task_t *next = bt->next_done;
        parsec_gpu_task_t *gpu_task = bt->gpu_task;
        parsec_data_copy_t *held[MAX_PARAM_COUNT];
        if( NULL != next ) { B200_PF(next); B200_PF(next->gpu_task); }
        const int nheld = b200_epilog_flows(dev, bt, held);
        (void)__parsec_complete_execution(es, gpu_task->ec);
        for( int i = 0; i < nheld; i++ ) (void)parsec_atomic_fetch_dec_int32(&held[i]->readers);
        gpu_task->last_data_check_epoch = 0;
        gpu_task->release_device_task(gpu_task);
        b200_bt_free(bt);
        bt = next;
        n++;
    }
    if( dev->nb_stalled > 0 && !dev->retry_stalled ) dev->retry_stalled = 1;
    parsec_atomic_wmb();
    (void)parsec_atomic_fetch_add_int64(&dev->epilogs_done, n);
    b200_nvtx_pop();
    return PARSEC_HOOK_RETURN_ASYNC;
}

#define B200_EPILOG_BATCH 4
static inline void b200_close_batch(parsec_device_b200_module_t *dev)
{
    b200_task_t *bt = dev->batch_head;
    if( NULL == bt ) return;
    dev->batch_head = NULL; dev->batch_len = 0;
    PARSEC_LIST_ITEM_SINGLETON(&bt->proxy);
    if( NULL == dev->completion_ring ) dev->completion_ring = &bt->proxy;
    else parsec_list_item_ring_push((parsec_list_item_t*)dev->completion_ring, (parsec_list_item_t*)&bt->proxy);
}

static void b200_complete(parsec_device_b200_module_t *dev, parsec_execution_stream_t *es, b200_task_t *bt)
{
    dev->super.super.super.executed_tasks++;
    dev->completed_now++;
    if( parsec_b200_parallel_completion && !bt->has_complete_stage && !dev->complete_inline ) {
        dev->epilogs_started++;
        bt->next_done = dev->batch_head; dev->batch_head = bt;
        if( ++dev->batch_len >= B200_EPILOG_BATCH ) b200_close_batch(dev);
        return;
    }
    parsec_gpu_task_t *gpu_task = bt->gpu_task;
    parsec_data_copy_t *held[MAX_PARAM_COUNT];
    const int nheld = b200_epilog_flows(dev, bt, held);
    if( NULL != gpu_task->complete_stage ) {
        parsec_gpu_task_t *gt = gpu_task;
        (void)gpu_task->complete_stage(&dev->super.super, &gt, &dev->lane->super);
    }
    __parsec_complete_execution(es, gpu_task->ec);
    for( int i = 0; i < nheld; i++ ) (void)parsec_atomic_fetch_dec_int32(&held[i]->readers);
    gpu_task->last_data_check_epoch = 0;
    gpu_task->release_device_task(gpu_task);
    b200_bt_free(bt);
}

static int b200_dma_pushout(parsec_device_b200_module_t *dev, b200_task_t *bt)
{
    parsec_gpu_task_t *gpu_task = bt->gpu_task;
    int n = 0;
    if( dev->dry_run ) return 0;
    b200_cuda_here(dev);
    if( NULL != gpu_task->stage_out && gpu_task->stage_out != parsec_default_gpu_stage_out ) {
        if( PARSEC_SUCCESS != gpu_task->stage_out(gpu_task, bt->dma_out_mask, &dev->lane->super) ) return 0;
        B200_CUDA(cudaEventRecord(b200_bt_event(dev, bt), dev->lane->cuda_stream), "cudaEventRecord", {});
        return 1;
    }
    for( uint32_t i = 0; i < gpu_task->nb_flows; i++ ) {
        if( !(bt->dma_out_mask & (1u << i)) ) continue;
        parsec_data_copy_t *gpu_copy = gpu_task->ec->data[i].data_out;
        parsec_data_copy_t *cpu_copy = gpu_copy->original->device_copies[0];
        if( NULL == cpu_copy || NULL == cpu_copy->device_private ) continue;
        B200_CUDA(cudaMemcpyAsync(cpu_copy->device_private, gpu_copy->device_private, gpu_task->flow_info[i].flow_span,
                                  cudaMemcpyDeviceToHost, dev->dma_stream), "pushout cudaMemcpyAsync", { continue; });
        dev->st.bytes_d2h_dma += gpu_task->flow_info[i].flow_span;
        n++;
    }
    if( n ) B200_CUDA(cudaEventRecord(b200_bt_event(dev, bt), dev->dma_stream), "cudaEventRecord", {});
    return n;
}

static void b200_build_cmd(parsec_device_b200_module_t *dev, b200_task_t *bt)
{
    parsec_gpu_task_t *gpu_task = bt->gpu_task;
    pb2_task_t *t = &bt->cmd;
    memset(t, 0, sizeof *t);
    t->body = (uint8_t)bt->body; t->nb_flows = (uint8_t)bt->nb_args;
    for( int a = 0; a < PB2_MAX_FLOWS; a++ ) t->tile[a] = -1;
    for( int a = 0; a < bt->nb_args; a++ ) {
        const int f = bt->arg_flow[a];
        const parsec_flow_t *flow = gpu_task->flow_info[f].flow;
        parsec_data_copy_t *out = gpu_task->ec->data[f].data_out;
        t->tile[a] = b200_tile_of(dev, out);
        t->access[a] = (uint8_t)(flow->flow_flags & PARSEC_FLOW_ACCESS_MASK);
        if( (gpu_task->pushout & (1 << f)) && (PARSEC_FLOW_ACCESS_WRITE & flow->flow_flags) ) {
            parsec_data_copy_t *cpu = out->original->device_copies[0];
            if( !bt->custom_stage && NULL != cpu && NULL != cpu->device_private &&
                NULL != b200_device_visible(cpu->device_private, gpu_task->flow_info[f].flow_span) && !(bt->peer_src_mask & (1u << f)) )
                t->access[a] |= PB2_FLOW_PUSHOUT;
            else bt->dma_out_mask |= (1u << f);
        }
    }
    for( uint32_t f = 0; f < gpu_task->nb_flows; f++ ) {
        int named = 0;
        for( int a = 0; a < bt->nb_args; a++ ) named |= (bt->arg_flow[a] == (int)f);
        if( !named && (gpu_task->pushout & (1 << f)) && (PARSEC_FLOW_ACCESS_WRITE & gpu_task->flow_info[f].flow->flow_flags) &&
            NULL != gpu_task->ec->data[f].data_out ) bt->dma_out_mask |= (1u << f);
    }
    t->iparam[0] = bt->iparam[0]; t->iparam[1] = bt->iparam[1]; t->iparam[2] = bt->iparam[2]; t->fparam = bt->fparam;
    t->locals[0] = gpu_task->ec->locals[0].value; t->locals[1] = gpu_task->ec->locals[1].value;
    bt->cmd_built = 1;
}

static int b200_push_engine(parsec_device_b200_module_t *dev, b200_task_t *bt)
{
    if( !bt->cmd_built ) b200_build_cmd(dev, bt);
    const int32_t state_before = bt->state;
    bt->state = BT_INFLIGHT;
    int rc = pb2_stream_submit(dev->stream, &bt->cmd, (uint64_t)(uintptr_t)bt, &bt->ticket);
    if( PB2_SUCCESS != rc ) {
        bt->state = state_before;
        if( PB2_ERR_OUT_OF_RESOURCE == rc ) return PARSEC_HOOK_RETURN_AGAIN;
        parsec_warning("device_b200: submit failed: %s", pb2_stream_last_error(dev->stream));
        return PARSEC_HOOK_RETURN_ERROR;
    }
    dev->n_engine++;
    return PARSEC_HOOK_RETURN_DONE;
}

static int b200_prepare_resident(parsec_device_b200_module_t *dev, b200_task_t *bt)
{
    parsec_gpu_task_t *gpu_task = bt->gpu_task;
    parsec_task_t *this_task = gpu_task->ec;
    const uint8_t my = dev->super.super.super.device_index;
    if( NULL == dev->tile_described ) return 0;
    for( uint32_t i = 0; i < gpu_task->nb_flows; i++ ) {
        const parsec_flow_t *flow = gpu_task->flow_info[i].flow;
        if( PARSEC_FLOW_ACCESS_NONE == (PARSEC_FLOW_ACCESS_MASK & flow->flow_flags) ) continue;
        const parsec_data_copy_t *in = this_task->data[i].data_in;
        if( NULL == in ) continue;
        if( in->device_index != my || NULL == in->device_private || NULL == in->original ) return 0;
        if( !dev->tile_described[b200_tile_of(dev, in)] ) return 0;
    }
    for( uint32_t i = 0; i < gpu_task->nb_flows; i++ ) {
        const parsec_flow_t *flow = gpu_task->flow_info[i].flow;
        const uint8_t type = (uint8_t)(flow->flow_flags & PARSEC_FLOW_ACCESS_MASK);
        if( PARSEC_FLOW_ACCESS_NONE == type ) { gpu_task->flow_info[i].flow_span = 0; continue; }
        parsec_data_copy_t *in = this_task->data[i].data_in;
        if( NULL == in ) continue;
        this_task->data[i].data_out = in;
        gpu_task->flow_info[i].source = NULL;
        if( PARSEC_FLOW_ACCESS_WRITE & type ) {
            in->version++;
            b200_lru_take(dev, in, 1);
            parsec_atomic_lock(&in->original->lock);
            in->original->owner_device = my; in->coherency_state = PARSEC_DATA_COHERENCY_OWNED;
            parsec_atomic_unlock(&in->original->lock);
        }
        if( PARSEC_FLOW_ACCESS_READ & type ) (void)parsec_atomic_fetch_inc_int32(&in->readers);
    }
    b200_build_cmd(dev, bt);
    bt->prepared = 1;
    return 1;
}

static int b200_chore_allows_batch(const parsec_task_t *task, const parsec_device_module_t *device)
{
    if( NULL == task || NULL == task->task_class || task->selected_chore < 0 ) return 0;
    const __parsec_chore_t *chore = &task->task_class->incarnations[task->selected_chore];
    return parsec_mca_device_type_supports_batch(device->type) && (0 != (chore->type & device->type)) &&
           (0 != (chore->type & PARSEC_DEV_CHORE_ALLOW_BATCH));
}

static int b200_lane_after_submit(parsec_device_b200_module_t *dev, b200_task_t *bt)
{
    parsec_gpu_task_t *gpu_task = bt->gpu_task;
    for( uint32_t i = 0; i < gpu_task->nb_flows; i++ )
        if( (gpu_task->pushout & (1 << i)) && (PARSEC_FLOW_ACCESS_WRITE & gpu_task->flow_info[i].flow->flow_flags) && NULL != gpu_task->ec->data[i].data_out ) {
            if( NULL != gpu_task->stage_out && gpu_task->stage_out != parsec_default_gpu_stage_out ) {
                if( PARSEC_SUCCESS != gpu_task->stage_out(gpu_task, 1u << i, &dev->lane->super) ) return PARSEC_HOOK_RETURN_ERROR;
            } else {
                parsec_data_copy_t *g = gpu_task->ec->data[i].data_out, *c = g->original->device_copies[0];
                if( NULL != c && NULL != c->device_private )
                    B200_CUDA(cudaMemcpyAsync(c->device_private, g->device_private, gpu_task->flow_info[i].flow_span, cudaMemcpyDeviceToHost, dev->lane->cuda_stream),
                              "lane pushout", { return PARSEC_HOOK_RETURN_ERROR; });
                dev->st.bytes_d2h_dma += gpu_task->flow_info[i].flow_span;
            }
        }
    B200_CUDA(cudaEventRecord(b200_bt_event(dev, bt), dev->lane->cuda_stream), "cudaEventRecord", {});
    bt->state = BT_LANE;
    dev->n_lane++;
    parsec_list_nolock_push_back(&dev->waiting_event, &bt->item);
    return PARSEC_HOOK_RETURN_DONE;
}

static int b200_lane_submit(parsec_device_b200_module_t *dev, b200_task_t *bt)
{
    parsec_gpu_task_t *gpu_task = bt->gpu_task;
    PARSEC_LIST_ITEM_SINGLETON(&gpu_task->list_item);
    b200_tl_recording = bt;
    int src = gpu_task->submit(&dev->super.super, gpu_task, &dev->lane->super);
    b200_tl_recording = NULL;
    bt->has_complete_stage = (NULL != gpu_task->complete_stage);
    if( src < 0 && PARSEC_HOOK_RETURN_ASYNC != src ) return PARSEC_HOOK_RETURN_ERROR;
    if( bt->body >= 0 ) {
        parsec_b200_submit_set_engine(gpu_task->submit);
        for( uint32_t i = 0; i < gpu_task->nb_flows; i++ ) {
            parsec_data_copy_t *out = gpu_task->ec->data[i].data_out;
            if( NULL == out || NULL == gpu_task->ec->data[i].data_in ) continue;
            pb2_tile_t tile; memset(&tile, 0, sizeof tile);
            tile.dev_ptr = out->device_private; tile.bytes = (uint32_t)gpu_task->flow_info[i].flow_span; tile.state = PB2_TILE_VALID;
            const uint8_t type = (uint8_t)(gpu_task->flow_info[i].flow->flow_flags & PARSEC_FLOW_ACCESS_MASK);
            tile.version = (PARSEC_FLOW_ACCESS_WRITE & type) ? out->version - 1 : out->version;
            parsec_data_copy_t *cpu = out->original->device_copies[0];
            tile.src_ptr = (NULL != cpu && NULL != cpu->device_private) ? b200_device_visible(cpu->device_private, tile.bytes) : NULL;
            (void)pb2_stream_set_tile(dev->stream, b200_tile_of(dev, out), &tile);
            dev->tile_described[b200_tile_of(dev, out)] = 1;
        }
        B200_CUDA(cudaEventRecord(b200_bt_event(dev, bt), dev->lane->cuda_stream), "cudaEventRecord", {});
        bt->state = BT_DMA_IN;
        parsec_list_nolock_push_back(&dev->waiting_event, &bt->item);
        return PARSEC_HOOK_RETURN_DONE;
    }
    parsec_list_item_t *ring = (parsec_list_item_t*)gpu_task->list_item.list_next;
    while( ring != &gpu_task->list_item ) {
        parsec_list_item_t *next = (parsec_list_item_t*)ring->list_next;
        parsec_gpu_task_t *member = (parsec_gpu_task_t*)ring;
        PARSEC_LIST_ITEM_SINGLETON(ring);
        dev->lane_pending--; dev->st.lane_batched++;
        if( PARSEC_HOOK_RETURN_DONE != b200_lane_after_submit(dev, B200_BT(member)) ) return PARSEC_HOOK_RETURN_ERROR;
        ring = next;
    }
    PARSEC_LIST_ITEM_SINGLETON(&gpu_task->list_item);
    return b200_lane_after_submit(dev, bt);
}

static int b200_fire_lane(parsec_device_b200_module_t *dev)
{
    int n = 0;
    while( dev->lane_pending > 0 ) {
        parsec_gpu_task_t *head = (parsec_gpu_task_t*)parsec_list_nolock_pop_front(dev->lane->super.fifo_pending);
        if( NULL == head ) { dev->lane_pending = 0; break; }
        dev->lane_pending--;
        if( PARSEC_HOOK_RETURN_DONE != b200_lane_submit(dev, B200_BT(head)) ) return -1;
        n++;
    }
    return n;
}

static int b200_start_task(parsec_device_b200_module_t *dev, parsec_execution_stream_t *es, b200_task_t *bt)
{
    parsec_gpu_task_t *gpu_task = bt->gpu_task;
    int rc;
    (void)es;
    dev->again_window = 0;
    if( bt->prepared ) { bt->state = BT_STAGED; return b200_push_engine(dev, bt); }
    if( dev->cold_inflight >= (int64_t)parsec_b200_stage_window && b200_needs_memory(dev, gpu_task) ) { dev->again_window = 1; return PARSEC_HOOK_RETURN_AGAIN; }
    uint64_t c0 = B200_TSC(), c1;
    if( PARSEC_HOOK_RETURN_DONE != (rc = b200_reserve(dev, bt)) ) return rc;
    c1 = B200_TSC(); dev->tsc_start[0] += c1 - c0; c0 = c1;

    const int custom_stage = (NULL != gpu_task->stage_in && gpu_task->stage_in != parsec_default_gpu_stage_in) ||
                             (NULL != gpu_task->stage_out && gpu_task->stage_out != parsec_default_gpu_stage_out);
    const parsec_task_class_t *tc = gpu_task->ec->task_class;
    bt->custom_stage = custom_stage;
    int known_engine = bt->recorded || dev->dry_run || (!custom_stage && parsec_b200_submit_is_engine(gpu_task->submit));

    if( known_engine ) {
        rc = b200_stage_in(dev, bt, 0);
        if( rc < 0 ) return rc;
        c1 = B200_TSC(); dev->tsc_start[1] += c1 - c0; c0 = c1;
        if( bt->cold_bytes ) (void)parsec_atomic_fetch_add_int64(&dev->cold_inflight, (int64_t)bt->cold_bytes);
        int src = 0;
        if( !bt->recorded ) {
            b200_tl_recording = bt;
            src = gpu_task->submit(&dev->super.super, gpu_task, &dev->lane->super);
            b200_tl_recording = NULL;
            bt->recorded = 1;
            bt->has_complete_stage = (NULL != gpu_task->complete_stage);
        }
        if( dev->dry_run && bt->body < 0 ) { bt->body = PB2_BODY_NOP; bt->nb_args = 0; }
        if( src < 0 || bt->body < 0 ) {
            parsec_warning("device_b200: body of task class %s stopped naming an engine body", tc ? tc->name : "?");
            return PARSEC_HOOK_RETURN_ERROR;
        }
        if( rc > 0 ) {
            B200_CUDA(cudaEventRecord(b200_bt_event(dev, bt), dev->dma_stream), "cudaEventRecord", {});
            bt->state = BT_DMA_IN;
            parsec_list_nolock_push_back(&dev->waiting_event, &bt->item);
            return PARSEC_HOOK_RETURN_DONE;
        }
        bt->state = BT_STAGED;
        c1 = B200_TSC(); dev->tsc_start[2] += c1 - c0; c0 = c1;
        rc = b200_push_engine(dev, bt);
        dev->tsc_start[3] += B200_TSC() - c0;
        return rc;
    }

    b200_cuda_here(dev);
    const int user_in = (NULL != gpu_task->stage_in && gpu_task->stage_in != parsec_default_gpu_stage_in);
    rc = b200_stage_in(dev, bt, user_in ? 2 : 1);
    if( rc < 0 ) return rc;
    if( bt->cold_bytes ) (void)parsec_atomic_fetch_add_int64(&dev->cold_inflight, (int64_t)bt->cold_bytes);
    if( user_in ) {
        uint32_t mask = 0;
        for( uint32_t i = 0; i < gpu_task->nb_flows; i++ )
            if( NULL != gpu_task->ec->data[i].data_out && PARSEC_DATA_STATUS_UNDER_TRANSFER == gpu_task->ec->data[i].data_out->data_transfer_status ) mask |= (1u << i);
        if( mask && PARSEC_SUCCESS != gpu_task->stage_in(gpu_task, mask, &dev->lane->super) ) return PARSEC_HOOK_RETURN_ERROR;
    }
    if( b200_chore_allows_batch(gpu_task->ec, &dev->super.super.super) && !parsec_b200_submit_is_engine(gpu_task->submit) ) {
        bt->state = BT_LANE;
        PARSEC_LIST_ITEM_SINGLETON(&gpu_task->list_item);
        parsec_list_nolock_push_back(dev->lane->super.fifo_pending, &gpu_task->list_item);
        dev->lane_pending++;
        return PARSEC_HOOK_RETURN_DONE;
    }
    return b200_lane_submit(dev, bt);
}

#define B200_SUBMIT_SET 256
static void * volatile b200_engine_submits[B200_SUBMIT_SET];
static int parsec_b200_submit_is_engine(parsec_advance_task_function_t fn)
{
    uintptr_t h = ((uintptr_t)fn >> 4) % B200_SUBMIT_SET;
    for( int p = 0; p < B200_SUBMIT_SET; p++ ) {
        void *v = b200_engine_submits[(h + p) % B200_SUBMIT_SET];
        if( v == (void*)fn ) return 1;
        if( NULL == v ) return 0;
    }
    return 0;
}
static void parsec_b200_submit_set_engine(parsec_advance_task_function_t fn)
{
    uintptr_t h = ((uintptr_t)fn >> 4) % B200_SUBMIT_SET;
    for( int p = 0; p < B200_SUBMIT_SET; p++ ) {
        void * volatile *slot = &b200_engine_submits[(h + p) % B200_SUBMIT_SET];
        if( *slot == (void*)fn ) return;
        if( NULL == *slot && parsec_atomic_cas_ptr(slot, NULL, (void*)fn) ) return;
    }
}

static const parsec_flow_t b200_prefetch_flow = {
    .name = "FLOW", .flow_flags = PARSEC_FLOW_ACCESS_READ, .flow_index = 0,
};
static parsec_task_class_t b200_prefetch_tc = {
    .name = "b200 data prefetch", .flags = 0, .task_class_id = 0, .nb_flows = 1, .nb_parameters = 0, .nb_locals = 0,
    .in = { &b200_prefetch_flow, NULL }, .out = { NULL },
};
static int b200_prefetch_submit(parsec_device_gpu_module_t *gpu_device, parsec_gpu_task_t *gpu_task, parsec_gpu_exec_stream_t *gpu_stream)
{
    static const int flow0 = 0;
    return parsec_b200_task_body(gpu_device, gpu_task, gpu_stream, PB2_BODY_NOP, 1, &flow0, NULL, 0.f);
}
static void b200_release_pseudo_task(parsec_gpu_task_t *gpu_task)
{
    if( NULL != gpu_task->ec ) {
        if( NULL != gpu_task->ec->data[0].data_in ) PARSEC_DATA_COPY_RELEASE(gpu_task->ec->data[0].data_in);
        free(gpu_task->ec);
        gpu_task->ec = NULL;
    }
    PARSEC_OBJ_RELEASE(gpu_task);
}

static parsec_hook_return_t b200_kernel_scheduler(parsec_device_module_t *module, parsec_execution_stream_t *es, void *_gpu_task);

static int b200_data_advise(parsec_device_module_t *module, parsec_data_t *data, int advice)
{
    switch( advice ) {
    case PARSEC_DEV_DATA_ADVICE_PREFERRED_DEVICE:
        data->preferred_device = module->device_index;
        return PARSEC_SUCCESS;
    case PARSEC_DEV_DATA_ADVICE_PREFETCH:
    case PARSEC_DEV_DATA_ADVICE_WARMUP: {
        parsec_data_copy_t *src = (data->owner_device >= 0) ? data->device_copies[data->owner_device] : data->device_copies[0];
        if( NULL == src ) return PARSEC_ERR_NOT_FOUND;
        parsec_gpu_task_t *gpu_task = (parsec_gpu_task_t*)PARSEC_OBJ_NEW(parsec_gpu_dsl_task_t);
        gpu_task->task_type = (PARSEC_DEV_DATA_ADVICE_PREFETCH == advice) ? PARSEC_GPU_TASK_TYPE_PREFETCH : PARSEC_GPU_TASK_TYPE_WARMUP;
        gpu_task->ec = (parsec_task_t*)calloc(1, sizeof(parsec_task_t));
        PARSEC_OBJ_CONSTRUCT(gpu_task->ec, parsec_task_t);
        gpu_task->ec->task_class = &b200_prefetch_tc;
        gpu_task->ec->selected_device = module;
        gpu_task->nb_flows = 1;
        gpu_task->flow_info[0].flow = &b200_prefetch_flow;
        gpu_task->flow_info[0].flow_span = data->span;
        gpu_task->stage_in = parsec_default_gpu_stage_in;
        gpu_task->stage_out = parsec_default_gpu_stage_out;
        gpu_task->submit = b200_prefetch_submit;
        gpu_task->release_device_task = b200_release_pseudo_task;
        PARSEC_DATA_COPY_RETAIN(src);
        gpu_task->ec->data[0].data_in = src;
        (void)b200_kernel_scheduler(module, NULL, gpu_task);
        return PARSEC_SUCCESS;
    }
    default:
        return PARSEC_ERR_NOT_FOUND;
    }
}

static void b200_finish(parsec_device_b200_module_t *dev, parsec_execution_stream_t *es, b200_task_t *bt)
{
    if( bt->cold_bytes ) { (void)parsec_atomic_fetch_add_int64(&dev->cold_inflight, -(int64_t)bt->cold_bytes); bt->cold_bytes = 0; }
    if( !dev->retry_stalled ) dev->retry_stalled = 1;
    if( bt->is_kernel ) { b200_complete(dev, es, bt); return; }
    parsec_gpu_task_t *gpu_task = bt->gpu_task;
    parsec_data_copy_t *out = gpu_task->ec->data[0].data_out;
    if( NULL != out ) {
        parsec_atomic_lock(&out->original->lock);
        if( PARSEC_DATA_STATUS_UNDER_TRANSFER == out->data_transfer_status ) {
            out->data_transfer_status = PARSEC_DATA_STATUS_COMPLETE_TRANSFER;
            parsec_data_end_transfer_ownership_to_copy(out->original, dev->super.super.super.device_index, PARSEC_FLOW_ACCESS_READ);
        }
        if( bt->peer_src_mask & 1u ) (void)parsec_atomic_fetch_dec_int32(&bt->peer_src[0]->readers);
        if( 1 == out->readers ) b200_lru_touch(dev, out);
        (void)parsec_atomic_fetch_dec_int32(&out->readers);
        parsec_atomic_unlock(&out->original->lock);
    }
    b200_bt_free(bt);
    gpu_task->last_data_check_epoch = 0;
    gpu_task->release_device_task(gpu_task);
    dev->completed_now++;
}

static parsec_device_b200_module_t *b200_forward_peer(parsec_device_b200_module_t *dev, const parsec_gpu_task_t *gpu_task)
{
    const uint8_t my = dev->super.super.super.device_index;
    parsec_device_b200_module_t *peer = NULL;
    if( PARSEC_GPU_TASK_TYPE_KERNEL != gpu_task->task_type ) return NULL;
    for( uint32_t i = 0; i < gpu_task->nb_flows; i++ ) {
        const parsec_flow_t *flow = gpu_task->flow_info[i].flow;
        if( PARSEC_FLOW_ACCESS_NONE == (PARSEC_FLOW_ACCESS_MASK & flow->flow_flags) ) continue;
        const parsec_data_copy_t *in = gpu_task->ec->data[i].data_in;
        if( NULL == in || in->device_index == my ) continue;
        if( !parsec_mca_device_is_gpu(in->device_index) ) {
            if( NULL != PARSEC_DATA_GET_COPY(in->original, my) ) continue;
            return NULL;
        }
        parsec_device_module_t *m = parsec_mca_device_get(in->device_index);
        if( !parsec_b200_is_b200_device(m) ) return NULL;
        if( NULL != peer && (parsec_device_module_t*)peer != m ) return NULL;
        peer = (parsec_device_b200_module_t*)m;
    }
    if( NULL == peer || peer->dry_run != dev->dry_run || b200_needs_memory(peer, gpu_task) ) return NULL;
    return peer;
}

static int b200_hand_back(parsec_device_b200_module_t *dev, parsec_execution_stream_t *es, b200_task_t *bt)
{
    parsec_device_b200_module_t *peer;
    if( NULL == es || BT_NEW != bt->state || NULL == (peer = b200_forward_peer(dev, bt->gpu_task)) ) return 0;
    parsec_gpu_task_t *gt = bt->gpu_task;
    parsec_task_t *task = gt->ec;
    parsec_list_nolock_remove(&dev->stalled, &bt->item);
    PARSEC_LIST_ITEM_SINGLETON(&bt->item);
    dev->nb_stalled--;
    b200_bt_free(bt);
    gt->last_data_check_epoch = UINT64_MAX;
    gt->release_device_task(gt);
    (void)parsec_atomic_fetch_add_int64(&task->selected_device->device_load, -task->load);
    task->selected_device = &peer->super.super.super;
    (void)parsec_atomic_fetch_add_int32(&dev->handed_back, 1);
    dev->st.forwarded++;
    b200_nvtx_mark("b200 task handed back to the runtime for a peer device");
    PARSEC_LIST_ITEM_SINGLETON(&task->super);
    (void)__parsec_reschedule(es, task);
    return 1;
}

static int b200_drain_inbox(parsec_device_b200_module_t *dev)
{
    int64_t head = dev->inbox_head;
    const int64_t head0 = head;
    for(;;) {
        b200_task_t * volatile *slot = &dev->inbox_ring[head & (B200_INBOX_SLOTS - 1)];
        b200_task_t *bt = *slot;
        if( NULL == bt ) break;
        parsec_atomic_rmb();
        *slot = NULL;
        head++;
        {
            const char *la = (const char*)dev->inbox_ring[(head + 6) & (B200_INBOX_SLOTS - 1)];
            if( NULL != la ) { B200_PFW(la); B200_PFW(la + 64); B200_PF(la + offsetof(b200_task_t, cmd)); }
        }
        for( int k = 0; k < bt->ntdesc; k++ )
            if( PB2_SUCCESS != pb2_stream_set_tile(dev->stream, bt->tdesc[k].tile, &bt->tdesc[k].desc) ) return -1;
        bt->ntdesc = 0; bt->defer_tiles = 0;
        switch( bt->prepared ) {
        case 1:  parsec_list_nolock_push_back(&dev->settled, &bt->item); dev->nb_settled++; dev->n_settled_by_caller++; break;
        case 2:  parsec_list_nolock_push_back(&dev->cold_q, &bt->item); dev->nb_cold++; dev->n_settled_by_caller++; break;
        case 3:  bt->state = BT_DMA_IN; parsec_list_nolock_push_back(&dev->waiting_event, &bt->item);
                 if( bt->cold_bytes ) (void)parsec_atomic_fetch_add_int64(&dev->cold_inflight, (int64_t)bt->cold_bytes);
                 break;
        default: parsec_list_nolock_push_back(&dev->stalled, &bt->item); dev->nb_stalled++; break;
        }
    }
    if( head != head0 ) { dev->inbox_head = head; dev->retry_stalled = 1; }
    return (int)(head - head0);
}

static int b200_start_pass(parsec_device_b200_module_t *dev, parsec_execution_stream_t *es)
{
    uint64_t t0 = B200_TSC(), t1;
    int moved = 0;
    {
        const int n = b200_drain_inbox(dev);
        if( n < 0 ) return -1;
        moved += n;
    }
    t1 = B200_TSC(); dev->tsc_s[0] += t1 - t0; t0 = t1;
    int started = 0;
    if( dev->retry_stalled && (dev->nb_settled > 0 || dev->nb_stalled > 0 || dev->nb_cold > 0) ) {
        int ring_full = 0, cut = 0;
        dev->retry_stalled = 0;
        while( dev->nb_settled > 0 ) {
            if( started >= 512 ) { cut = 1; break; }
            b200_task_t *bt = (b200_task_t*)PARSEC_LIST_ITERATOR_FIRST(&dev->settled);
            parsec_list_item_t *la = PARSEC_LIST_ITERATOR_NEXT(&bt->item);
            if( la != PARSEC_LIST_ITERATOR_END(&dev->settled) ) { la = PARSEC_LIST_ITERATOR_NEXT(la);
                if( la != PARSEC_LIST_ITERATOR_END(&dev->settled) ) { B200_PF(la); B200_PF((const char*)la + offsetof(b200_task_t, cmd)); } }
            parsec_list_nolock_remove(&dev->settled, &bt->item);
            PARSEC_LIST_ITEM_SINGLETON(&bt->item);
            if( BT_NEW == bt->state ) bt->state = BT_STAGED;
            const int rc = b200_push_engine(dev, bt);
            if( PARSEC_HOOK_RETURN_AGAIN == rc ) { parsec_list_nolock_push_front(&dev->settled, &bt->item); ring_full = 1; break; }
            if( PARSEC_HOOK_RETURN_DONE != rc ) return -1;
            dev->nb_settled--;
            started++;
        }
        while( !ring_full && !cut && dev->nb_cold > 0 ) {
            if( started >= 512 ) { cut = 1; break; }
            b200_task_t *bt = (b200_task_t*)PARSEC_LIST_ITERATOR_FIRST(&dev->cold_q);
            if( bt->cold_bytes && dev->cold_inflight >= (int64_t)parsec_b200_stage_window ) break;
            parsec_list_nolock_remove(&dev->cold_q, &bt->item);
            PARSEC_LIST_ITEM_SINGLETON(&bt->item);
            if( BT_NEW == bt->state ) bt->state = BT_STAGED;
            const uint64_t cold = bt->cold_bytes;
            const int rc = b200_push_engine(dev, bt);
            if( PARSEC_HOOK_RETURN_AGAIN == rc ) { parsec_list_nolock_push_front(&dev->cold_q, &bt->item); ring_full = 1; break; }
            if( PARSEC_HOOK_RETURN_DONE != rc ) return -1;
            if( cold ) (void)parsec_atomic_fetch_add_int64(&dev->cold_inflight, (int64_t)cold);
            dev->nb_cold--;
            started++;
        }
        parsec_list_item_t *it = PARSEC_LIST_ITERATOR_FIRST(&dev->stalled), *next;
        int mem_blocked = 0;
        for( ; !ring_full && !cut && it != PARSEC_LIST_ITERATOR_END(&dev->stalled); it = next ) {
            b200_task_t *bt = (b200_task_t*)it;
            next = PARSEC_LIST_ITERATOR_NEXT(it);
            int rc;
            if( started >= 512 ) { cut = 1; break; }
            if( next != PARSEC_LIST_ITERATOR_END(&dev->stalled) ) {
                parsec_list_item_t *la = next;
                b200_pf4((b200_task_t*)la); la = PARSEC_LIST_ITERATOR_NEXT(la);
                if( la != PARSEC_LIST_ITERATOR_END(&dev->stalled) ) { b200_pf3((b200_task_t*)la); la = PARSEC_LIST_ITERATOR_NEXT(la);
                if( la != PARSEC_LIST_ITERATOR_END(&dev->stalled) ) { b200_pf2((b200_task_t*)la); la = PARSEC_LIST_ITERATOR_NEXT(la);
                if( la != PARSEC_LIST_ITERATOR_END(&dev->stalled) ) { b200_pf1((b200_task_t*)la); } } }
            }
            if( mem_blocked && BT_NEW == bt->state && b200_needs_memory(dev, bt->gpu_task) ) {
                if( b200_hand_back(dev, es, bt) ) moved++;
                continue;
            }
            parsec_list_nolock_remove(&dev->stalled, it);
            PARSEC_LIST_ITEM_SINGLETON(it);
            if( BT_NEW == bt->state ) {
                b200_lock(&dev->alloc_lock);
                const int n = b200_drain_inbox(dev);
                rc = (n < 0) ? PARSEC_HOOK_RETURN_ERROR : b200_start_task(dev, es, bt);
                b200_unlock(&dev->alloc_lock);
                if( n > 0 ) moved += n;
            } else rc = b200_push_engine(dev, bt);
            if( PARSEC_HOOK_RETURN_AGAIN == rc ) {
                if( next == PARSEC_LIST_ITERATOR_END(&dev->stalled) ) parsec_list_nolock_push_back(&dev->stalled, it);
                else parsec_list_nolock_add_before(&dev->stalled, next, it);
                if( BT_NEW != bt->state ) break;
                if( dev->again_window ) break;
                if( b200_hand_back(dev, es, bt) ) { moved++; continue; }
                mem_blocked = 1;
                continue;
            }
            if( PARSEC_HOOK_RETURN_DONE != rc ) return -1;
            dev->nb_stalled--;
            started++;
        }
        if( cut ) dev->retry_stalled = 1;
    }
    if( dev->lane_pending > 0 ) { const int n = b200_fire_lane(dev); if( n < 0 ) return -1; moved += n; }
    if( started && PB2_SUCCESS != pb2_stream_kick(dev->stream) ) return -1;
    t1 = B200_TSC(); dev->tsc_s[1] += t1 - t0; t0 = t1;
    if( !parsec_list_nolock_is_empty(&dev->waiting_event) ) {
        parsec_list_item_t *it = PARSEC_LIST_ITERATOR_FIRST(&dev->waiting_event), *next;
        for( ; it != PARSEC_LIST_ITERATOR_END(&dev->waiting_event); it = next ) {
            b200_task_t *bt = (b200_task_t*)it;
            next = PARSEC_LIST_ITERATOR_NEXT(it);
            cudaError_t q = cudaEventQuery(bt->ev);
            if( cudaErrorNotReady == q ) { (void)cudaGetLastError(); continue; }
            if( cudaSuccess != q ) { parsec_warning("device_b200: event failed: %s", cudaGetErrorString(q)); return -1; }
            parsec_list_nolock_remove(&dev->waiting_event, it);
            PARSEC_LIST_ITEM_SINGLETON(it);
            if( BT_DMA_IN == bt->state ) {
                parsec_gpu_task_t *gt = bt->gpu_task;
                for( uint32_t i = 0; i < gt->nb_flows; i++ ) {
                    parsec_data_copy_t *out = gt->ec->data[i].data_out;
                    if( NULL == out || NULL == gt->ec->data[i].data_in || PARSEC_DATA_STATUS_UNDER_TRANSFER != out->data_transfer_status ) continue;
                    parsec_atomic_lock(&out->original->lock);
                    out->data_transfer_status = PARSEC_DATA_STATUS_COMPLETE_TRANSFER;
                    parsec_data_end_transfer_ownership_to_copy(out->original, dev->super.super.super.device_index,
                                                               (uint8_t)(gt->flow_info[i].flow->flow_flags & PARSEC_FLOW_ACCESS_MASK));
                    parsec_atomic_unlock(&out->original->lock);
                }
                bt->state = BT_STAGED;
                int rc = b200_push_engine(dev, bt);
                if( PARSEC_HOOK_RETURN_AGAIN == rc ) { parsec_list_nolock_push_front(&dev->stalled, &bt->item); dev->nb_stalled++; dev->retry_stalled = 1; }
                else if( PARSEC_HOOK_RETURN_DONE != rc ) return -1;
                else if( PB2_SUCCESS != pb2_stream_kick(dev->stream) ) return -1;
            } else {
                b200_task_t *old;
                do { old = dev->lane_done; bt->next_done = old; } while( !parsec_atomic_cas_ptr(&dev->lane_done, old, bt) );
            }
            moved++;
        }
    }
    t1 = B200_TSC(); dev->tsc_s[2] += t1 - t0; t0 = t1;
    return moved + started;
}

static void b200_trace_task(parsec_device_b200_module_t *dev, const b200_task_t *bt, const pb2_retire_t *r)
{
    if( dev->trace_n == dev->trace_cap ) {
        dev->trace_cap = dev->trace_cap ? 2 * dev->trace_cap : 65536;
        dev->trace_ev = (b200_trace_ev_t*)realloc(dev->trace_ev, dev->trace_cap * sizeof(b200_trace_ev_t));
    }
    b200_trace_ev_t *e = &dev->trace_ev[dev->trace_n++];
    const parsec_task_t *t = bt->gpu_task->ec;
    memset(e, 0, sizeof *e);
    snprintf(e->name, sizeof e->name, "%s", (NULL != t && NULL != t->task_class && NULL != t->task_class->name) ? t->task_class->name : "?");
    if( NULL != t ) { e->locals[0] = t->locals[0].value; e->locals[1] = t->locals[1].value; }
    e->body = bt->body; e->smid = (int32_t)r->smid; e->t_start_ns = r->t_start_ns; e->t_end_ns = r->t_end_ns; e->cold_bytes = bt->cold_bytes;
}

static void b200_trace_write(parsec_device_b200_module_t *dev)
{
    if( NULL == dev->trace_ev || 0 == dev->trace_n || NULL == parsec_b200_trace || '\0' == parsec_b200_trace[0] ) return;
    char path[1024];
    snprintf(path, sizeof path, "%s.%d.json", parsec_b200_trace, (int)dev->super.super.super.device_index);
    FILE *f = fopen(path, "w");
    if( NULL == f ) { parsec_warning("device_b200: cannot write the trace %s", path); return; }
    uint64_t t0 = UINT64_MAX;
    for( size_t i = 0; i < dev->trace_n; i++ ) if( dev->trace_ev[i].t_start_ns && dev->trace_ev[i].t_start_ns < t0 ) t0 = dev->trace_ev[i].t_start_ns;
    fprintf(f, "{\"displayTimeUnit\": \"ns\", \"traceEvents\": [\n");
    for( size_t i = 0; i < dev->trace_n; i++ ) {
        const b200_trace_ev_t *e = &dev->trace_ev[i];
        fprintf(f, "%s{\"name\": \"%s\", \"ph\": \"X\", \"pid\": %d, \"tid\": %d, \"ts\": %.3f, \"dur\": %.3f, "
                   "\"args\": {\"l0\": %d, \"l1\": %d, \"body\": %d, \"stage_in_bytes\": %lu}}",
                i ? ",\n" : "", e->name, (int)dev->super.super.super.device_index, e->smid,
                (double)(e->t_start_ns - t0) * 1e-3, (double)(e->t_end_ns - e->t_start_ns) * 1e-3,
                e->locals[0], e->locals[1], e->body, (unsigned long)e->cold_bytes);
    }
    fprintf(f, "\n]}\n");
    fclose(f);
}

static int b200_retire_pass(parsec_device_b200_module_t *dev, parsec_execution_stream_t *es)
{
    uint64_t t0 = B200_TSC(), t1;
    if( dev->fatal ) return -1;
    if( NULL != dev->lane_done ) {
        b200_task_t *bt = dev->lane_done;
        while( !parsec_atomic_cas_ptr(&dev->lane_done, bt, NULL) ) bt = dev->lane_done;
        while( NULL != bt ) { b200_task_t *next = bt->next_done; b200_finish(dev, es, bt); bt = next; }
    }
    if( !parsec_list_nolock_is_empty(&dev->waiting_out) ) {
        parsec_list_item_t *it = PARSEC_LIST_ITERATOR_FIRST(&dev->waiting_out), *next;
        for( ; it != PARSEC_LIST_ITERATOR_END(&dev->waiting_out); it = next ) {
            b200_task_t *bt = (b200_task_t*)it;
            next = PARSEC_LIST_ITERATOR_NEXT(it);
            cudaError_t q = cudaEventQuery(bt->ev);
            if( cudaErrorNotReady == q ) { (void)cudaGetLastError(); continue; }
            if( cudaSuccess != q ) { parsec_warning("device_b200: event failed: %s", cudaGetErrorString(q)); return -1; }
            parsec_list_nolock_remove(&dev->waiting_out, it);
            PARSEC_LIST_ITEM_SINGLETON(it);
            b200_finish(dev, es, bt);
        }
    }
    for(;;) {
        int n = pb2_stream_poll(dev->stream, dev->retbuf, (int32_t)(sizeof(dev->retbuf) / sizeof(dev->retbuf[0])));
        if( n < 0 ) { parsec_warning("device_b200: %s", pb2_stream_last_error(dev->stream)); return -1; }
        t1 = B200_TSC(); dev->tsc[n ? 3 : 5] += t1 - t0; t0 = t1;
        dev->complete_inline = (1 == n) && (0 == pb2_stream_inflight(dev->stream)) && (dev->inbox_tail == dev->inbox_head);
        if( n > 0 ) b200_nvtx_push("b200 retire pass");
        for( int i = 0; i < n; i++ ) {
            b200_task_t *bt = (b200_task_t*)(uintptr_t)dev->retbuf[i].cookie;
            if( i + 5 < n ) { const char *la = (const char*)(uintptr_t)dev->retbuf[i + 5].cookie; B200_PFW(la); B200_PFW(la + 64); B200_PFW(la + offsetof(b200_task_t, proxy)); }
            if( NULL == bt->gpu_task || BT_INFLIGHT != bt->state ) {
                parsec_warning("device_b200: retire record %d/%d for a task that is not in flight (bt %p state %d ticket %d/%d gpu_task %p)",
                               i, n, (void*)bt, bt->state, bt->ticket, dev->retbuf[i].ticket, (void*)bt->gpu_task);
                return -1;
            }
            bt->result = dev->retbuf[i].result;
            if( NULL != dev->trace_ev || (NULL != parsec_b200_trace && '\0' != parsec_b200_trace[0]) ) b200_trace_task(dev, bt, &dev->retbuf[i]);
            if( (PB2_BODY_CHECK_I32 == bt->body || PB2_BODY_CHECK_F32 == bt->body) && (bt->result >> 32) ) dev->st.check_mismatches += bt->result >> 32;
            bt->ticket = -1;
            if( PB2_SUCCESS != dev->retbuf[i].status ) { parsec_warning("device_b200: task ran an unknown engine body"); return -1; }
            if( bt->dma_out_mask && b200_dma_pushout(dev, bt) > 0 ) {
                bt->state = BT_DMA_OUT;
                parsec_list_nolock_push_back(&dev->waiting_out, &bt->item);
            } else b200_finish(dev, es, bt);
        }
        if( n > 0 ) b200_nvtx_pop();
        t1 = B200_TSC(); dev->tsc[4] += t1 - t0; t0 = t1;
        if( n < (int)(sizeof(dev->retbuf) / sizeof(dev->retbuf[0])) ) break;
    }
    dev->complete_inline = 0;
    b200_close_batch(dev);
    return 0;
}

static inline int b200_start_work(const parsec_device_b200_module_t *dev)
{
    return dev->inbox_tail != dev->inbox_head ||
           ((dev->nb_stalled > 0 || dev->nb_settled > 0 || dev->nb_cold > 0) && dev->retry_stalled) ||
           !parsec_list_nolock_is_empty((parsec_list_t*)&dev->waiting_event);
}

static int b200_try_start(parsec_device_b200_module_t *dev, parsec_execution_stream_t *es, int sticky)
{
    for(;;) {
        if( dev->starter_active || !parsec_atomic_cas_int32(&dev->starter_active, 0, 1) ) return 0;
        int rc;
        do { b200_nvtx_push("b200 start pass"); rc = b200_start_pass(dev, es); b200_nvtx_pop(); } while( rc > 0 && sticky );
        if( rc < 0 ) dev->fatal = 1;
        parsec_atomic_wmb();
        dev->starter_active = 0;
        parsec_mfence();
        if( rc < 0 ) return -1;
        if( dev->inbox_tail == dev->inbox_head ) return 0;
    }
}


static parsec_hook_return_t
b200_kernel_scheduler(parsec_device_module_t *module, parsec_execution_stream_t *es, void *_gpu_task)
{
    parsec_device_b200_module_t *dev = (parsec_device_b200_module_t*)module;
    parsec_gpu_task_t *gpu_task = (parsec_gpu_task_t*)_gpu_task;

    if( 0 == dev->first_entry_ns ) dev->first_entry_ns = b200_now_ns();
    int32_t inside = parsec_atomic_fetch_inc_int32(&dev->callers_inside) + 1;
    if( inside > dev->max_callers_inside ) dev->max_callers_inside = inside;
    if( UINT64_MAX != gpu_task->last_data_check_epoch ) {
        parsec_warning("device_b200: gpu_task %p handed to kernel_scheduler twice (epoch %lx)", (void*)gpu_task, (unsigned long)gpu_task->last_data_check_epoch);
        abort();
    }
    b200_task_t *bt = b200_bt_new(dev, gpu_task);
    bt->proxy.taskpool = (NULL != gpu_task->ec) ? gpu_task->ec->taskpool : NULL;
    bt->custom_stage = (NULL != gpu_task->stage_in && gpu_task->stage_in != parsec_default_gpu_stage_in) ||
                       (NULL != gpu_task->stage_out && gpu_task->stage_out != parsec_default_gpu_stage_out);
    if( !bt->custom_stage && NULL != gpu_task->submit && (dev->dry_run || parsec_b200_submit_is_engine(gpu_task->submit)) ) {
        b200_tl_recording = bt;
        const int src = gpu_task->submit(&dev->super.super, gpu_task, &dev->lane->super);
        b200_tl_recording = NULL;
        if( src >= 0 && bt->body >= 0 ) bt->recorded = 1;
        else if( !dev->dry_run ) bt->body = -1;
        else { bt->recorded = 1; bt->body = PB2_BODY_NOP; bt->nb_args = 0; }
    }
    bt->has_complete_stage = (NULL != gpu_task->complete_stage);
    int decided = 0;
    if( bt->recorded && bt->is_kernel && !b200_prepare_resident(dev, bt) && dev->nb_stalled < 64 && !dev->memory_pressure &&
        dev->inbox_tail - dev->inbox_head < B200_INBOX_SLOTS - 4096  ) {
        b200_lock(&dev->alloc_lock);
        decided = 1;
        bt->defer_tiles = 1;
        if( PARSEC_HOOK_RETURN_DONE == b200_reserve(dev, bt) ) {
            const int rc = b200_stage_in(dev, bt, 0);
            if( 0 == rc ) { b200_build_cmd(dev, bt); bt->prepared = 2; }
            else if( rc > 0 ) {
                B200_CUDA(cudaEventRecord(b200_bt_event(dev, bt), dev->dma_stream), "cudaEventRecord", {});
                bt->prepared = 3;
            } else if( PARSEC_HOOK_RETURN_AGAIN != rc ) dev->fatal = 1;
        }
        if( 0 == bt->prepared ) bt->defer_tiles = (bt->ntdesc > 0);
    }
    int32_t before = parsec_atomic_fetch_add_int32(&dev->owed, 1);
    {
        const int64_t idx = parsec_atomic_fetch_add_int64(&dev->inbox_tail, 1);
        while( idx - dev->inbox_head >= B200_INBOX_SLOTS ) { _mm_pause(); }
        parsec_atomic_wmb();
        dev->inbox_ring[idx & (B200_INBOX_SLOTS - 1)] = bt;
    }
    if( decided ) b200_unlock(&dev->alloc_lock);
    (void)parsec_atomic_fetch_dec_int32(&dev->callers_inside);
    if( before > 0 ) {
        (void)b200_try_start(dev, es, 1);
        return PARSEC_HOOK_RETURN_ASYNC;
    }

    dev->st.manager_entries++;
    b200_nvtx_mark("b200 manager elected");
    if( 0 == dev->first_task_ns ) dev->first_task_ns = b200_now_ns();
    if( NULL == es ) {
        es = parsec_my_execution_stream();
        if( NULL == es && NULL != module->context ) es = module->context->virtual_processes[0]->execution_streams[0];
    }
    b200_cuda_here(dev);
    uint64_t idle_spins = 0;
    for(;;) {
        dev->completed_now = 0;
        if( 0 == (++idle_spins & 0x3ffffff) && NULL != getenv("PARSEC_B200_DEBUG") ) {
            fprintf(stderr, "b200 manager stuck? owed %d inbox %ld stalled %d settled %d starter %d retry %d stream inflight %d executed %lu\n",
                    dev->owed, (long)(dev->inbox_tail - dev->inbox_head), dev->nb_stalled, dev->nb_settled, dev->starter_active, dev->retry_stalled,
                    pb2_stream_inflight(dev->stream), (unsigned long)module->executed_tasks);
        }
        if( (dev->nb_stalled > 0 || dev->nb_settled > 0 || dev->nb_cold > 0) && ++dev->blocked_spins >= 1024 ) {
            dev->blocked_spins = 0; dev->retry_stalled = 1;
        }
        if( b200_start_work(dev) && b200_try_start(dev, es, 0) < 0 ) dev->fatal = 1;
        if( b200_retire_pass(dev, es) < 0 ) {
            parsec_warning("GPU[%d:%s]: the device engine reported a fatal error; giving up", module->device_index, module->name);
            return PARSEC_HOOK_RETURN_DISABLE;
        }
        if( NULL != dev->completion_ring ) {
            parsec_task_t *ring = dev->completion_ring;
            dev->completion_ring = NULL;
            const uint64_t ts0 = B200_TSC();
            __parsec_schedule(es, ring, 0);
            dev->tsc[6] += B200_TSC() - ts0;
        }
        int32_t done_now = dev->completed_now;
        if( dev->handed_back ) done_now += parsec_atomic_fetch_and_int32(&dev->handed_back, 0);
        if( done_now ) {
            idle_spins = 0;
            const int32_t left = parsec_atomic_fetch_sub_int32(&dev->owed, done_now) - done_now;
            if( 0 == left ) { dev->last_done_ns = b200_now_ns(); return PARSEC_HOOK_RETURN_ASYNC; }
            if( left < 0 ) {
                parsec_warning("GPU[%d:%s]: more tasks completed than were handed over (%d)", module->device_index, module->name, left);
                return PARSEC_HOOK_RETURN_DISABLE;
            }
        }
    }
}

static int b200_set_device(parsec_device_gpu_module_t *gpu)
{
    parsec_device_b200_module_t *dev = B200_DEV(gpu);
    if( dev->dry_run ) return PARSEC_SUCCESS;
    B200_CUDA(cudaSetDevice(dev->super.cuda_index), "cudaSetDevice", { return PARSEC_ERROR; });
    return PARSEC_SUCCESS;
}
static int b200_memory_info(parsec_device_gpu_module_t *gpu, size_t *free_mem, size_t *total_mem)
{
    parsec_device_b200_module_t *dev = B200_DEV(gpu);
    if( dev->dry_run ) { *free_mem = *total_mem = (size_t)8 << 30; return PARSEC_SUCCESS; }
    pb2_engine_info_t info;
    if( PB2_SUCCESS != pb2_engine_info(dev->engine, &info) ) return PARSEC_ERROR;
    *free_mem = info.free_mem; *total_mem = info.total_mem;
    return PARSEC_SUCCESS;
}
static int b200_memory_allocate(parsec_device_gpu_module_t *gpu, size_t bytes, void **addr)
{
    parsec_device_b200_module_t *dev = B200_DEV(gpu);
    if( dev->dry_run ) { *addr = (void*)((uintptr_t)1 << 40); dev->slab_base = (char*)*addr; return PARSEC_SUCCESS; }
    if( PB2_SUCCESS != pb2_engine_malloc(dev->engine, bytes, addr) ) return PARSEC_ERR_OUT_OF_RESOURCE;
    dev->slab_base = (char*)*addr;
    return PARSEC_SUCCESS;
}
static int b200_memory_free(parsec_device_gpu_module_t *gpu, void *addr)
{
    parsec_device_b200_module_t *dev = B200_DEV(gpu);
    if( dev->dry_run ) return PARSEC_SUCCESS;
    return (PB2_SUCCESS == pb2_engine_free(dev->engine, addr)) ? PARSEC_SUCCESS : PARSEC_ERROR;
}
static void *b200_find_incarnation(parsec_device_gpu_module_t *gpu, const char *fname)
{
    (void)gpu;
    return parsec_device_find_function(fname, NULL, NULL);
}

static int b200_memory_register(parsec_device_module_t *device, parsec_data_collection_t *desc, void *ptr, size_t length)
{
    parsec_device_b200_module_t *dev = (parsec_device_b200_module_t*)device;
    if( desc->memory_registration_status == PARSEC_MEMORY_STATUS_REGISTERED ) return PARSEC_SUCCESS;
    void *alias = ptr;
    int revived = 0;
    parsec_atomic_lock(&b200_ranges_lock);
    for( int i = 0; i < b200_nb_ranges; i++ ) {
        b200_host_range_t *r = &b200_ranges[i];
        if( !r->lazy ) continue;
        if( r->base == (char*)ptr && r->len >= length ) { r->lazy = 0; revived = 1; break; }
        if( (char*)ptr < r->base + r->len && r->base < (char*)ptr + length ) {
            char *old = r->base;
            *r = b200_ranges[--b200_nb_ranges]; i--;
            if( !dev->dry_run ) { (void)pb2_stream_quiesce(dev->stream); (void)pb2_engine_host_unregister(dev->engine, old); }
        }
    }
    parsec_atomic_unlock(&b200_ranges_lock);
    if( revived ) { dev->st.registration_hits++; desc->memory_registration_status = PARSEC_MEMORY_STATUS_REGISTERED; return PARSEC_SUCCESS; }
    if( !dev->dry_run ) {
        if( PB2_SUCCESS != pb2_engine_host_register(dev->engine, ptr, length, &alias) ) return PARSEC_ERROR;
    }
    parsec_atomic_lock(&b200_ranges_lock);
    if( b200_nb_ranges == b200_cap_ranges ) {
        b200_cap_ranges = b200_cap_ranges ? 2 * b200_cap_ranges : 16;
        b200_ranges = (b200_host_range_t*)realloc(b200_ranges, sizeof(b200_host_range_t) * (size_t)b200_cap_ranges);
    }
    b200_ranges[b200_nb_ranges].base = (char*)ptr; b200_ranges[b200_nb_ranges].len = length; b200_ranges[b200_nb_ranges].alias = (char*)alias;
    b200_ranges[b200_nb_ranges].lazy = 0;
    b200_nb_ranges++;
    parsec_atomic_unlock(&b200_ranges_lock);
    desc->memory_registration_status = PARSEC_MEMORY_STATUS_REGISTERED;
    return PARSEC_SUCCESS;
}

static int b200_memory_unregister(parsec_device_module_t *device, parsec_data_collection_t *desc, void *ptr)
{
    parsec_device_b200_module_t *dev = (parsec_device_b200_module_t*)device;
    if( desc->memory_registration_status == PARSEC_MEMORY_STATUS_UNREGISTERED ) return PARSEC_SUCCESS;
    int found = 0;
    parsec_atomic_lock(&b200_ranges_lock);
    for( int i = 0; i < b200_nb_ranges; i++ ) {
        if( b200_ranges[i].base != (char*)ptr || b200_ranges[i].lazy ) continue;
        if( parsec_b200_registration_cache ) b200_ranges[i].lazy = 1;
        else { b200_ranges[i] = b200_ranges[--b200_nb_ranges]; found = 1; }
        break;
    }
    parsec_atomic_unlock(&b200_ranges_lock);
    if( found && !dev->dry_run ) {
        (void)pb2_stream_quiesce(dev->stream);
        (void)pb2_engine_host_unregister(dev->engine, ptr);
    }
    desc->memory_registration_status = PARSEC_MEMORY_STATUS_UNREGISTERED;
    return PARSEC_SUCCESS;
}

static void b200_registration_cache_drop(parsec_device_b200_module_t *dev)
{
    parsec_atomic_lock(&b200_ranges_lock);
    for( int i = 0; i < b200_nb_ranges; i++ ) {
        if( !b200_ranges[i].lazy ) continue;
        if( !dev->dry_run ) (void)pb2_engine_host_unregister(dev->engine, b200_ranges[i].base);
        b200_ranges[i] = b200_ranges[--b200_nb_ranges]; i--;
    }
    parsec_atomic_unlock(&b200_ranges_lock);
}

static void b200_profile_print(parsec_device_b200_module_t *dev)
{
    if( NULL == getenv("PARSEC_B200_PROFILE") ) return;
    uint64_t tot = 0; for( int i = 3; i < 7; i++ ) tot += dev->tsc[i];
    fprintf(stderr, "b200 starter Mcycles: inbox %.1f start %.1f events %.1f (total %.1f, %lu settled by their caller) | manager Mcycles: poll %.1f finish %.1f idle-poll %.1f schedule %.1f (total %.1f, %lu tasks so far, %lu manager entries)\n",
            dev->tsc_s[0] * 1e-6, dev->tsc_s[1] * 1e-6, dev->tsc_s[2] * 1e-6, (dev->tsc_s[0] + dev->tsc_s[1] + dev->tsc_s[2]) * 1e-6, (unsigned long)dev->n_settled_by_caller,
            dev->tsc[3] * 1e-6, dev->tsc[4] * 1e-6, dev->tsc[5] * 1e-6, dev->tsc[6] * 1e-6,
            tot * 1e-6, (unsigned long)dev->super.super.super.executed_tasks, (unsigned long)dev->st.manager_entries);
    memset(dev->tsc_s, 0, sizeof dev->tsc_s);
    fprintf(stderr, "b200 manager start Mcycles: reserve %.1f stage-in %.1f record %.1f command %.1f\n",
            dev->tsc_start[0] * 1e-6, dev->tsc_start[1] * 1e-6, dev->tsc_start[2] * 1e-6, dev->tsc_start[3] * 1e-6);
    memset(dev->tsc, 0, sizeof dev->tsc); memset(dev->tsc_start, 0, sizeof dev->tsc_start);
}

static int b200_memory_release(parsec_device_module_t *device)
{
    parsec_device_b200_module_t *dev = (parsec_device_b200_module_t*)device;
    b200_profile_print(dev);
    dev->first_task_ns = dev->first_entry_ns = 0;
    while( dev->epilogs_done < dev->epilogs_started ) { parsec_atomic_rmb(); }
    if( !dev->dry_run ) (void)pb2_stream_quiesce(dev->stream);
    while( b200_write_back_some(dev, 64) > 0 ) { }
    const int rc = parsec_device_flush_lru(device);
    dev->memory_pressure = 0;
    if( NULL != dev->tile_described ) memset(dev->tile_described, 0, (size_t)dev->super.super.mem_nb_blocks);
    return rc;
}

static int b200_all_devices_attached(parsec_device_module_t *device)
{
    parsec_device_b200_module_t *dev = (parsec_device_b200_module_t*)device, *peer;
    dev->super.super.peer_access_mask = (int16_t)(1 << device->device_index);
    if( dev->dry_run ) {
        for( int j = 0; NULL != (peer = (parsec_device_b200_module_t*)parsec_device_b200_component.modules[j]); j++ )
            dev->super.super.peer_access_mask = (int16_t)(dev->super.super.peer_access_mask | (1 << peer->super.super.super.device_index));
        return PARSEC_SUCCESS;
    }
    for( int j = 0; NULL != (peer = (parsec_device_b200_module_t*)parsec_device_b200_component.modules[j]); j++ ) {
        if( peer == dev ) continue;
        if( PB2_SUCCESS == pb2_engine_enable_peer(dev->engine, peer->super.cuda_index) )
            dev->super.super.peer_access_mask = (int16_t)(dev->super.super.peer_access_mask | (1 << peer->super.super.super.device_index));
        else parsec_warning("GPU[%d:%s]: no peer access to %s: its replicas will be fetched through the copy engine",
                            device->device_index, device->name, peer->super.super.super.name);
    }
    return PARSEC_SUCCESS;
}

int parsec_b200_get_stats(const parsec_device_module_t *device, parsec_b200_stats_t *stats)
{
    if( !parsec_b200_is_b200_device(device) || NULL == stats ) return PARSEC_ERR_BAD_PARAM;
    parsec_device_b200_module_t *dev = (parsec_device_b200_module_t*)device;
    pb2_stream_stats_t ss;
    *stats = dev->st;
    stats->tasks_engine = dev->n_engine; stats->tasks_lane = dev->n_lane;
    stats->first_entry_ns = dev->first_entry_ns; stats->first_task_ns = dev->first_task_ns; stats->last_done_ns = dev->last_done_ns;
    stats->max_concurrent_callers = (uint64_t)dev->max_callers_inside;
    if( PB2_SUCCESS == pb2_stream_stats(dev->stream, &ss) ) {
        stats->kernel_launches = ss.kernel_launches; stats->released_on_device = ss.released_on_device;
        stats->bytes_h2d_kernel = ss.bytes_h2d; stats->bytes_d2d_kernel = ss.bytes_d2d; stats->bytes_d2h_kernel = ss.bytes_d2h;
    }
    return PARSEC_SUCCESS;
}

int parsec_b200_module_init(int dev_id, parsec_device_module_t **module)
{
    parsec_device_b200_module_t *dev = NULL;
    if( 0 != posix_memalign((void**)&dev, 64, sizeof(parsec_device_b200_module_t)) ) return PARSEC_ERR_OUT_OF_RESOURCE;
    memset(dev, 0, sizeof(parsec_device_b200_module_t));
    parsec_device_gpu_module_t *gpu = &dev->super.super;
    parsec_device_module_t *device = &gpu->super;
    *module = NULL;
    PARSEC_OBJ_CONSTRUCT(device, parsec_device_module_t);
    dev->dry_run = parsec_b200_dry_run > 0;
    dev->super.cuda_index = (uint8_t)dev_id;
    dev->super.major = 9; dev->super.minor = 0;
    if( -1 == asprintf(&device->name, "b200(%d)", dev_id) ) { free(dev); return PARSEC_ERROR; }

    if( !dev->dry_run ) {
        pb2_engine_params_t ep;
        memset(&ep, 0, sizeof ep);
        if( PB2_SUCCESS != pb2_engine_create(&dev->engine, dev_id, &ep) ) {
            parsec_warning("device_b200: CUDA device %d is not usable by the engine (needs sm_90)", dev_id);
            free(device->name); free(dev);
            return PARSEC_ERR_DEVICE;
        }
        B200_CUDA(cudaSetDevice(dev_id), "cudaSetDevice", {});
        B200_CUDA(cudaStreamCreateWithFlags(&dev->dma_stream, cudaStreamNonBlocking), "cudaStreamCreate", {});
    }
    gpu->max_exec_streams = 1;
    gpu->exec_stream = (parsec_gpu_exec_stream_t**)malloc(sizeof(parsec_gpu_exec_stream_t*));
    dev->lane = (parsec_cuda_exec_stream_t*)calloc(1, sizeof(parsec_cuda_exec_stream_t));
    gpu->exec_stream[0] = &dev->lane->super;
    gpu->num_exec_streams = 1;
    if( !dev->dry_run ) B200_CUDA(cudaStreamCreateWithFlags(&dev->lane->cuda_stream, cudaStreamNonBlocking), "cudaStreamCreate", {});
    PARSEC_OBJ_CONSTRUCT(&dev->lane->super.infos, parsec_info_object_array_t);
    parsec_info_object_array_init(&dev->lane->super.infos, &parsec_per_stream_infos, &dev->lane->super);
    dev->lane->super.fifo_pending = (parsec_list_t*)PARSEC_OBJ_NEW(parsec_list_t);
    if( -1 == asprintf(&dev->lane->super.name, "b200(%d)", dev_id) ) dev->lane->super.name = NULL;

    device->type                 = PARSEC_DEV_CUDA;
    device->attach               = parsec_device_attach;
    device->detach               = parsec_device_detach;
    device->taskpool_register    = parsec_device_taskpool_register;
    device->taskpool_unregister  = parsec_device_taskpool_unregister;
    device->memory_register      = b200_memory_register;
    device->memory_unregister    = b200_memory_unregister;
    device->memory_release       = b200_memory_release;
    device->data_advise          = b200_data_advise;
    device->kernel_scheduler     = b200_kernel_scheduler;
    device->all_devices_attached = b200_all_devices_attached;
    gpu->set_device       = b200_set_device;
    gpu->memory_info      = b200_memory_info;
    gpu->memory_allocate  = b200_memory_allocate;
    gpu->memory_free      = b200_memory_free;
    gpu->find_incarnation = b200_find_incarnation;
    device->gflops_fp16 = 989000; device->gflops_tf32 = 495000; device->gflops_fp32 = 67000; device->gflops_fp64 = 34000;
    device->gflops_guess = 0;
    device->device_load = 0;

    PARSEC_OBJ_CONSTRUCT(&gpu->gpu_mem_lru, parsec_list_t);
    PARSEC_OBJ_CONSTRUCT(&gpu->gpu_mem_owned_lru, parsec_list_t);
    PARSEC_OBJ_CONSTRUCT(&gpu->pending, parsec_fifo_t);
    PARSEC_OBJ_CONSTRUCT(&dev->stalled, parsec_list_t);
    PARSEC_OBJ_CONSTRUCT(&dev->settled, parsec_list_t);
    PARSEC_OBJ_CONSTRUCT(&dev->waiting_out, parsec_list_t);
    PARSEC_OBJ_CONSTRUCT(&dev->cold_q, parsec_list_t);
    PARSEC_OBJ_CONSTRUCT(&dev->waiting_event, parsec_list_t);
    memset(&dev->lru_lock, 0, sizeof dev->lru_lock);
    dev->inbox_ring = (b200_task_t * volatile *)calloc(B200_INBOX_SLOTS, sizeof(b200_task_t*));

    int nblocks = parsec_b200_memory_number_of_blocks;
    if( dev->dry_run && -1 == nblocks ) nblocks = 4096;
    if( PARSEC_SUCCESS != parsec_device_memory_reserve(gpu, parsec_b200_memory_percentage, nblocks, (size_t)parsec_b200_memory_block_size) ) goto failed;

    dev->tile_described = (uint8_t*)calloc((size_t)gpu->mem_nb_blocks + 1, 1);
    pb2_stream_params_t sp;
    memset(&sp, 0, sizeof sp);
    sp.cmd_slots = parsec_b200_cmd_slots;
    sp.max_tiles = (int32_t)gpu->mem_nb_blocks;
    sp.idle_us = parsec_b200_idle_us;
    sp.dry_run = dev->dry_run;
    sp.max_workers = parsec_b200_max_workers;
    sp.trace = (NULL != parsec_b200_trace && '\0' != parsec_b200_trace[0]);
    if( parsec_b200_nvtx && NULL == b200_nvtx_domain ) b200_nvtx_domain = nvtxDomainCreateA("parsec_b200");
    if( PB2_SUCCESS != pb2_stream_create(dev->engine, &sp, &dev->stream) ) goto failed;
    *module = device;
    return PARSEC_SUCCESS;
failed:
    parsec_warning("device_b200: initialisation of device %d failed", dev_id);
    if( NULL != dev->engine ) pb2_engine_destroy(dev->engine);
    free(device->name); free(dev);
    return PARSEC_ERROR;
}

int parsec_b200_module_fini(parsec_device_module_t *device)
{
    parsec_device_b200_module_t *dev = (parsec_device_b200_module_t*)device;
    parsec_device_gpu_module_t *gpu = &dev->super.super;
    if( NULL != dev->stream ) { (void)pb2_stream_quiesce(dev->stream); }
    b200_profile_print(dev);
    b200_trace_write(dev);
    free(dev->trace_ev); dev->trace_ev = NULL; dev->trace_n = dev->trace_cap = 0;
    while( dev->epilogs_done < dev->epilogs_started ) { parsec_atomic_rmb(); }
    while( b200_write_back_some(dev, 64) > 0 ) { }
    parsec_device_memory_release(gpu);
    b200_registration_cache_drop(dev);
    if( NULL != dev->stream ) { pb2_stream_destroy(dev->stream); dev->stream = NULL; }
    free((void*)dev->inbox_ring); dev->inbox_ring = NULL;
    PARSEC_OBJ_DESTRUCT(&gpu->pending);
    PARSEC_OBJ_DESTRUCT(&dev->lane->super.infos);
    free(dev->lane->super.name);
    PARSEC_OBJ_RELEASE(dev->lane->super.fifo_pending);
    if( !dev->dry_run ) {
        (void)cudaStreamDestroy(dev->lane->cuda_stream);
        (void)cudaStreamDestroy(dev->dma_stream);
    }
    free(dev->tile_described);
    free(dev->lane); free(gpu->exec_stream);
    if( NULL != dev->engine ) { pb2_engine_destroy(dev->engine); dev->engine = NULL; }
    free(device->name); device->name = NULL;
    return PARSEC_SUCCESS;
}
```

Baseline: 99.33 million.

## Make stream submission thread-safe and let callers push ready tasks directly

```diff
diff --git a/parsec_b200/csrc/pb2_stream.cu b/parsec_b200/csrc/pb2_stream.cu
--- a/parsec_b200/csrc/pb2_stream.cu
+++ b/parsec_b200/csrc/pb2_stream.cu
@@ -341,9 +341,9 @@
     std::vector<void*> dev_allocs;
     cudaStream_t kstream = nullptr;
     int nworkers = 0;
-    unsigned long long cmd_written = 0;
-    unsigned long long consumed_seen = 0;
-    std::vector<int32_t> free_tickets, free_nodes;
+    alignas(64) std::atomic<uint64_t> cmd_reserved{0};
+    std::atomic<uint64_t> consumed_seen{0};
+    std::vector<int32_t> free_nodes;
     std::vector<uint64_t> cookie;
     std::vector<uint16_t> tk_parts;
     std::vector<std::vector<int32_t>> tk_nodes;
@@ -354,7 +354,7 @@
     alignas(64) std::atomic<uint64_t> freed_head{0};
     alignas(64) std::atomic<uint64_t> sub_tasks{0};
     std::atomic<uint64_t> sub_entries{0};
-    uint64_t ret_entries_seen = 0;
+    std::atomic<uint64_t> ret_entries_seen{0};
     alignas(64) std::atomic<uint64_t> ret_tasks{0};
     std::atomic<uint64_t> ret_entries{0};
     std::mutex launch_mu;
@@ -415,11 +415,13 @@
     s->e = e; s->p = p; s->dry = p.dry_run != 0;
     s->slots = round_pow2((uint32_t)p.cmd_slots, 1024u, 1u << 21);
     s->ring_cap = s->slots * 4u;
-    s->free_tickets.reserve(s->slots); s->free_nodes.reserve(s->slots);
-    for (int32_t i = (int32_t)s->slots - 1; i >= 0; --i) { s->free_tickets.push_back(i); s->free_nodes.push_back(i); }
+    s->free_nodes.reserve(s->slots);
+    for (int32_t i = (int32_t)s->slots - 1; i >= 0; --i) s->free_nodes.push_back(i);
     s->tile_bytes.assign((size_t)p.max_tiles, 0);
     s->cookie.assign(s->slots, 0); s->tk_parts.assign(s->slots, 1); s->tk_nodes.resize(s->slots); s->tk_live.assign(s->slots, 0);
-    s->freed.assign(s->slots, -1);
+    s->freed.resize(s->slots);
+    for (uint32_t i = 0; i < s->slots; ++i) s->freed[i] = (int32_t)i;
+    s->freed_tail.store(s->slots);
     if (s->dry) {
         s->dry_tasks.resize(s->slots);
         s->dry_tiles.resize((size_t)p.max_tiles);
@@ -520,42 +522,54 @@
     return PB2_SUCCESS;
 }
 
-static int stream_cmd_slot(pb2_stream_t* s, Cmd** out) {
-    if (s->cmd_written - s->consumed_seen >= (unsigned long long)s->slots) s->consumed_seen = s->h_ctl->cmd_consumed;
-    if (s->cmd_written - s->consumed_seen >= (unsigned long long)s->slots) {
-        int rc = stream_launch_if_parked(s);
-        if (rc != PB2_SUCCESS) return rc;
-        unsigned long long spins = 0;
-        while (s->cmd_written - s->h_ctl->cmd_consumed >= (unsigned long long)s->slots) {
-            if (s->h_ctl->state == HS_ERROR) { s->last_error = "streaming kernel aborted"; return PB2_ERR_DEVICE; }
-            if ((++spins & 0xfffff) == 0 && s->h_ctl->state == HS_STOPPED) { rc = stream_launch_if_parked(s); if (rc != PB2_SUCCESS) return rc; }
-        }
-        s->consumed_seen = s->h_ctl->cmd_consumed;
-    }
-    *out = &s->h_cmd[s->cmd_written & (s->slots - 1)];
-    __builtin_prefetch(&s->h_cmd[(s->cmd_written + 6) & (s->slots - 1)], 1, 3);
-    return PB2_SUCCESS;
-}
-static void stream_cmd_publish(pb2_stream_t* s, Cmd* c) {
-    const uint32_t gen = (uint32_t)(s->cmd_written / (unsigned long long)s->slots) + 1u;
+static int stream_cmd_slot(pb2_stream_t* s, Cmd** out, uint64_t* idx_out) {
+    const uint64_t idx = s->cmd_reserved.fetch_add(1, std::memory_order_relaxed);
+    if (idx - s->consumed_seen.load(std::memory_order_relaxed) >= (uint64_t)s->slots) {
+        uint64_t consumed = s->h_ctl->cmd_consumed;
+        if (idx - consumed >= (uint64_t)s->slots) {
+            int rc = stream_launch_if_parked(s);
+            if (rc != PB2_SUCCESS) return rc;
+            unsigned long long spins = 0;
+            while (idx - (consumed = s->h_ctl->cmd_consumed) >= (uint64_t)s->slots) {
+                if (s->h_ctl->state == HS_ERROR) { s->last_error = "streaming kernel aborted"; return PB2_ERR_DEVICE; }
+                if ((++spins & 0xfffff) == 0 && s->h_ctl->state == HS_STOPPED) { rc = stream_launch_if_parked(s); if (rc != PB2_SUCCESS) return rc; }
+            }
+        }
+        s->consumed_seen.store(consumed, std::memory_order_relaxed);
+    }
+    *out = &s->h_cmd[idx & (s->slots - 1)];
+    *idx_out = idx;
+    return PB2_SUCCESS;
+}
+static void stream_cmd_publish(pb2_stream_t* s, Cmd* c, uint64_t idx) {
+    const uint32_t gen = (uint32_t)(idx / (uint64_t)s->slots) + 1u;
     std::atomic_thread_fence(std::memory_order_release);
     *reinterpret_cast<volatile uint32_t*>(&c->stamp) = gen;
-    s->cmd_written++;
+}
+
+static bool stream_take_ticket(pb2_stream_t* s, int32_t* tk) {
+    uint64_t h = s->freed_head.load(std::memory_order_relaxed);
+    for (;;) {
+        if (h == s->freed_tail.load(std::memory_order_acquire)) return false;
+        const int32_t v = s->freed[h & (s->slots - 1)];
+        if (s->freed_head.compare_exchange_weak(h, h + 1, std::memory_order_acq_rel, std::memory_order_relaxed)) { *tk = v; return true; }
+    }
 }
 
 int pb2_stream_set_tile(pb2_stream_t* s, int32_t tile, const pb2_tile_t* desc) {
     if (!s || !desc || tile < 0 || tile >= s->p.max_tiles) return PB2_ERR_BAD_PARAM;
     s->tile_bytes[(size_t)tile] = desc->bytes;
-    if (s->dry) { s->dry_tiles[(size_t)tile] = *desc; return PB2_SUCCESS; }
+    if (s->dry) { std::lock_guard<std::mutex> guard(s->dry_mu); s->dry_tiles[(size_t)tile] = *desc; return PB2_SUCCESS; }
     Cmd* c;
-    int rc = stream_cmd_slot(s, &c);
+    uint64_t idx;
+    int rc = stream_cmd_slot(s, &c, &idx);
     if (rc != PB2_SUCCESS) return rc;
     memset(c, 0, 60);
     c->op = CMD_TILE;
     c->u.tset.tile = tile; c->u.tset.state = desc->state; c->u.tset.version = desc->version; c->u.tset.src_kind = desc->src_kind;
     c->u.tset.dev_ptr = (uint64_t)(uintptr_t)desc->dev_ptr; c->u.tset.src_ptr = (uint64_t)(uintptr_t)desc->src_ptr;
     c->u.tset.bytes = desc->bytes;
-    stream_cmd_publish(s, c);
+    stream_cmd_publish(s, c, idx);
     return PB2_SUCCESS;
 }
 
@@ -567,39 +581,34 @@
     if (task->dep_goal < 0 || task->dep_goal > 0xffff) return PB2_ERR_VALUE_OUT_OF_BOUNDS;
     for (int f = 0; f < task->nb_flows; ++f)
         if (task->tile[f] >= s->p.max_tiles) { s->last_error = "tile id out of bounds"; return PB2_ERR_VALUE_OUT_OF_BOUNDS; }
-    if (s->free_tickets.empty()) {
-        uint64_t h = s->freed_head.load(std::memory_order_relaxed);
-        const uint64_t t = s->freed_tail.load(std::memory_order_acquire);
-        for (; h != t; ++h) s->free_tickets.push_back(s->freed[h & (s->slots - 1)]);
-        s->freed_head.store(h, std::memory_order_release);
-        if (s->free_tickets.empty()) return PB2_ERR_OUT_OF_RESOURCE;
-    }
     const uint32_t np = (uint32_t)task_parts(*task, [&](int32_t id) { return s->tile_bytes[(size_t)id]; },
                                              s->p.part_bytes, PB2_MAX_PARTS);
     {
-        const uint64_t sub = s->sub_entries.load(std::memory_order_relaxed);
-        if (sub - s->ret_entries_seen + np + 64 > (uint64_t)s->ring_cap / 2) {
-            s->ret_entries_seen = s->ret_entries.load(std::memory_order_acquire);
-            if (sub - s->ret_entries_seen + np + 64 > (uint64_t)s->ring_cap / 2) return PB2_ERR_OUT_OF_RESOURCE;
-        }
-    }
-    const int32_t tk = s->free_tickets.back();
+        const uint64_t sub = s->sub_entries.fetch_add(np, std::memory_order_relaxed) + np;
+        if (sub - s->ret_entries_seen.load(std::memory_order_relaxed) + 64 > (uint64_t)s->ring_cap / 2) {
+            const uint64_t seen = s->ret_entries.load(std::memory_order_acquire);
+            s->ret_entries_seen.store(seen, std::memory_order_relaxed);
+            if (sub - seen + 64 > (uint64_t)s->ring_cap / 2) {
+                s->sub_entries.fetch_sub(np, std::memory_order_relaxed);
+                return PB2_ERR_OUT_OF_RESOURCE;
+            }
+        }
+    }
+    int32_t tk;
+    if (!stream_take_ticket(s, &tk)) { s->sub_entries.fetch_sub(np, std::memory_order_relaxed); return PB2_ERR_OUT_OF_RESOURCE; }
+    s->cookie[(size_t)tk] = cookie; s->tk_parts[(size_t)tk] = (uint16_t)np; s->tk_live[(size_t)tk] = 1;
+    if (ticket) *ticket = tk;
     if (s->dry) {
         std::lock_guard<std::mutex> guard(s->dry_mu);
-        s->free_tickets.pop_back();
-        s->cookie[(size_t)tk] = cookie; s->tk_parts[(size_t)tk] = (uint16_t)np; s->tk_live[(size_t)tk] = 1;
-        s->sub_entries.store(s->sub_entries.load(std::memory_order_relaxed) + np, std::memory_order_relaxed);
-        s->sub_tasks.store(s->sub_tasks.load(std::memory_order_relaxed) + 1, std::memory_order_release);
-        if (ticket) *ticket = tk;
+        s->sub_tasks.fetch_add(1, std::memory_order_release);
         DryTask& dt = s->dry_tasks[(size_t)tk];
         dt.t = *task; dt.dep = task->dep_goal; dt.succ.clear(); dt.done = false;
         if (dt.dep == 0) s->dry_ready.push_back(tk);
     } else {
         Cmd* c;
-        int rc = stream_cmd_slot(s, &c);
+        uint64_t idx;
+        int rc = stream_cmd_slot(s, &c, &idx);
         if (rc != PB2_SUCCESS) return rc;
-        s->free_tickets.pop_back();
-        s->cookie[(size_t)tk] = cookie; s->tk_parts[(size_t)tk] = (uint16_t)np; s->tk_live[(size_t)tk] = 1;
         memset(c, 0, 60);
         c->op = CMD_TASK; c->body = task->body; c->nb_flows = task->nb_flows; c->flags = task->flags;
         c->nparts = (uint16_t)np; c->dep_goal = (uint16_t)task->dep_goal;
@@ -607,10 +616,8 @@
         for (int f = 0; f < PB2_MAX_FLOWS; ++f) { c->u.task.tile[f] = f < task->nb_flows ? task->tile[f] : -1; c->u.task.access[f] = task->access[f]; }
         c->u.task.iparam[0] = task->iparam[0]; c->u.task.iparam[1] = task->iparam[1]; c->u.task.iparam[2] = task->iparam[2];
         c->u.task.fparam = task->fparam; c->u.task.locals[0] = task->locals[0]; c->u.task.locals[1] = task->locals[1];
-        s->sub_entries.store(s->sub_entries.load(std::memory_order_relaxed) + np, std::memory_order_relaxed);
-        s->sub_tasks.store(s->sub_tasks.load(std::memory_order_relaxed) + 1, std::memory_order_release);
-        if (ticket) *ticket = tk;
-        stream_cmd_publish(s, c);
+        s->sub_tasks.fetch_add(1, std::memory_order_release);
+        stream_cmd_publish(s, c, idx);
     }
     return PB2_SUCCESS;
 }
@@ -618,33 +625,35 @@
 int pb2_stream_add_edge(pb2_stream_t* s, int32_t pred, int32_t succ) {
     if (!s || pred < 0 || succ < 0 || pred >= (int32_t)s->slots || succ >= (int32_t)s->slots) return PB2_ERR_BAD_PARAM;
     if (!s->tk_live[(size_t)pred] || !s->tk_live[(size_t)succ]) { s->last_error = "edge names a ticket that is not in flight"; return PB2_ERR_BAD_PARAM; }
-    s->st.edges++;
     if (s->dry) {
         std::lock_guard<std::mutex> guard(s->dry_mu);
+        s->st.edges++;
         DryTask& p = s->dry_tasks[(size_t)pred];
         if (p.done) { if (--s->dry_tasks[(size_t)succ].dep == 0) s->dry_ready.push_back(succ); }
         else p.succ.push_back(succ);
         return PB2_SUCCESS;
     }
-    Cmd* c;
-    int rc = stream_cmd_slot(s, &c);
-    if (rc != PB2_SUCCESS) return rc;
     int32_t node;
     {
         std::lock_guard<std::mutex> guard(s->nodes_mu);
         if (s->free_nodes.empty()) return PB2_ERR_OUT_OF_RESOURCE;
         node = s->free_nodes.back(); s->free_nodes.pop_back();
         s->tk_nodes[(size_t)pred].push_back(node);
-    }
+        s->st.edges++;
+    }
+    Cmd* c;
+    uint64_t idx;
+    int rc = stream_cmd_slot(s, &c, &idx);
+    if (rc != PB2_SUCCESS) return rc;
     memset(c, 0, 60);
     c->op = CMD_EDGE; c->u.edge.pred = pred; c->u.edge.succ = succ; c->u.edge.node = node;
-    stream_cmd_publish(s, c);
+    stream_cmd_publish(s, c, idx);
     return PB2_SUCCESS;
 }
 
 int pb2_stream_kick(pb2_stream_t* s) {
     if (!s) return PB2_ERR_BAD_PARAM;
-    if (s->dry || s->cmd_written == 0) return PB2_SUCCESS;
+    if (s->dry || s->cmd_reserved.load(std::memory_order_relaxed) == 0) return PB2_SUCCESS;
     return stream_launch_if_parked(s);
 }
 
@@ -727,13 +736,13 @@
     if (!s) return PB2_ERR_BAD_PARAM;
     if (s->dry) return PB2_SUCCESS;
     STREAM_CUDA(s, cudaSetDevice(s->e->cuda_device));
-    if (s->cmd_written != s->h_ctl->cmd_consumed) { int rc = stream_launch_if_parked(s); if (rc != PB2_SUCCESS) return rc; }
+    if (s->cmd_reserved.load() != s->h_ctl->cmd_consumed) { int rc = stream_launch_if_parked(s); if (rc != PB2_SUCCESS) return rc; }
     s->h_ctl->stop_req = 1;
     std::atomic_thread_fence(std::memory_order_seq_cst);
     STREAM_CUDA(s, cudaStreamSynchronize(s->kstream));
     s->h_ctl->stop_req = 0;
     if (s->h_ctl->state == HS_ERROR) { s->last_error = "streaming kernel aborted"; return PB2_ERR_DEVICE; }
-    if (s->cmd_written != s->h_ctl->cmd_consumed) return pb2_stream_quiesce(s);
+    if (s->cmd_reserved.load() != s->h_ctl->cmd_consumed) return pb2_stream_quiesce(s);
     return PB2_SUCCESS;
 }
 
diff --git a/parsec_b200/mca/b200/device_b200_module.c b/parsec_b200/mca/b200/device_b200_module.c
--- a/parsec_b200/mca/b200/device_b200_module.c
+++ b/parsec_b200/mca/b200/device_b200_module.c
@@ -86,8 +86,6 @@
     uint64_t             cold_bytes;
     struct parsec_device_b200_module_s *dev;
     int32_t              is_kernel;
-    int32_t              defer_tiles;
-    int32_t              ntdesc;
     pb2_task_t           cmd __attribute__((aligned(64)));
     parsec_task_t        proxy __attribute__((aligned(64)));
     int32_t              nb_args;
@@ -101,7 +99,6 @@
     int32_t              ev_dev;
     struct b200_task_s  *next_free;
     struct b200_task_s  *next_done;
-    struct { int32_t tile; pb2_tile_t desc; } tdesc[MAX_PARAM_COUNT];
 } b200_task_t;
 
 typedef struct b200_host_range_s { char *base; size_t len; char *alias; int lazy; } b200_host_range_t;
@@ -140,15 +137,14 @@
     volatile int64_t     cold_inflight B200_LINE;
     volatile int64_t     inbox_head B200_LINE;
     parsec_list_t        stalled B200_LINE;
-    parsec_list_t        settled;
     parsec_list_t        cold_q;
     int32_t              nb_cold;
     parsec_list_t        waiting_event;
-    int32_t              nb_settled;
     int32_t              nb_stalled;
     int32_t              again_window;
     int32_t              lane_pending;
-    uint64_t             n_engine, n_lane, n_settled_by_caller;
+    uint64_t             n_lane, n_started;
+    uint64_t             n_engine;
     uint64_t             tsc_start[4];
     uint64_t             tsc_s[3];
     parsec_list_t        waiting_out B200_LINE;
@@ -247,7 +243,7 @@
     bt->dev = dev;
     bt->gpu_task = gpu_task; bt->state = BT_NEW; bt->ticket = -1; bt->body = -1; bt->nb_args = 0;
     bt->peer_src_mask = 0; bt->dma_out_mask = 0; bt->result = 0; bt->custom_stage = 0; bt->cold_bytes = 0;
-    bt->recorded = 0; bt->has_complete_stage = 0; bt->prepared = 0; bt->cmd_built = 0; bt->defer_tiles = 0; bt->ntdesc = 0;
+    bt->recorded = 0; bt->has_complete_stage = 0; bt->prepared = 0; bt->cmd_built = 0;
     bt->is_kernel = (NULL == gpu_task) || (PARSEC_GPU_TASK_TYPE_KERNEL == gpu_task->task_type);
     if( NULL != gpu_task ) gpu_task->last_data_check_epoch = (uint64_t)(uintptr_t)bt;
     return bt;
@@ -529,12 +525,9 @@
     return 0;
 }
 
-static int b200_emit_tile(parsec_device_b200_module_t *dev, b200_task_t *bt, int32_t tid, const pb2_tile_t *tile)
-{
-    if( !bt->defer_tiles ) return (PB2_SUCCESS == pb2_stream_set_tile(dev->stream, tid, tile)) ? 0 : -1;
-    if( bt->ntdesc >= MAX_PARAM_COUNT ) return -1;
-    bt->tdesc[bt->ntdesc].tile = tid; bt->tdesc[bt->ntdesc].desc = *tile; bt->ntdesc++;
-    return 0;
+static int b200_emit_tile(parsec_device_b200_module_t *dev, int32_t tid, const pb2_tile_t *tile)
+{
+    return (PB2_SUCCESS == pb2_stream_set_tile(dev->stream, tid, tile)) ? 0 : -1;
 }
 
 static int b200_stage_in(parsec_device_b200_module_t *dev, b200_task_t *bt, int mode)
@@ -584,7 +577,7 @@
                 tile.version = (PARSEC_FLOW_ACCESS_WRITE & type) ? out->version - 1 : out->version;
                 if( NULL != original->device_copies[0] && NULL != original->device_copies[0]->device_private )
                     tile.src_ptr = b200_device_visible(original->device_copies[0]->device_private, span);
-                if( 0 != b200_emit_tile(dev, bt, b200_tile_of(dev, out), &tile) ) return PARSEC_HOOK_RETURN_ERROR;
+                if( 0 != b200_emit_tile(dev, b200_tile_of(dev, out), &tile) ) return PARSEC_HOOK_RETURN_ERROR;
                 dev->tile_described[b200_tile_of(dev, out)] = 1;
             }
             continue;
@@ -674,7 +667,7 @@
         if( !for_lane ) {
             const int32_t tid = b200_tile_of(dev, out);
             if( -1 != transfer_from || !dev->tile_described[tid] ) {
-                if( 0 != b200_emit_tile(dev, bt, tid, &tile) ) { parsec_atomic_unlock(&original->lock); return PARSEC_HOOK_RETURN_ERROR; }
+                if( 0 != b200_emit_tile(dev, tid, &tile) ) { parsec_atomic_unlock(&original->lock); return PARSEC_HOOK_RETURN_ERROR; }
                 dev->tile_described[tid] = 1;
             }
         }
@@ -905,8 +898,22 @@
         parsec_warning("device_b200: submit failed: %s", pb2_stream_last_error(dev->stream));
         return PARSEC_HOOK_RETURN_ERROR;
     }
-    dev->n_engine++;
     return PARSEC_HOOK_RETURN_DONE;
+}
+
+static int b200_submit_direct(parsec_device_b200_module_t *dev, b200_task_t *bt)
+{
+    const int64_t cold = (int64_t)bt->cold_bytes;
+    if( cold && parsec_atomic_fetch_add_int64(&dev->cold_inflight, cold) >= (int64_t)parsec_b200_stage_window ) {
+        (void)parsec_atomic_fetch_add_int64(&dev->cold_inflight, -cold);
+        return 0;
+    }
+    if( PARSEC_HOOK_RETURN_DONE != b200_push_engine(dev, bt) ) {
+        if( cold ) (void)parsec_atomic_fetch_add_int64(&dev->cold_inflight, -cold);
+        return 0;
+    }
+    if( PB2_SUCCESS != pb2_stream_kick(dev->stream) ) dev->fatal = 1;
+    return 1;
 }
 
 static int b200_prepare_resident(parsec_device_b200_module_t *dev, b200_task_t *bt)
@@ -1262,12 +1269,9 @@
             const char *la = (const char*)dev->inbox_ring[(head + 6) & (B200_INBOX_SLOTS - 1)];
             if( NULL != la ) { B200_PFW(la); B200_PFW(la + 64); B200_PF(la + offsetof(b200_task_t, cmd)); }
         }
-        for( int k = 0; k < bt->ntdesc; k++ )
-            if( PB2_SUCCESS != pb2_stream_set_tile(dev->stream, bt->tdesc[k].tile, &bt->tdesc[k].desc) ) return -1;
-        bt->ntdesc = 0; bt->defer_tiles = 0;
         switch( bt->prepared ) {
-        case 1:  parsec_list_nolock_push_back(&dev->settled, &bt->item); dev->nb_settled++; dev->n_settled_by_caller++; break;
-        case 2:  parsec_list_nolock_push_back(&dev->cold_q, &bt->item); dev->nb_cold++; dev->n_settled_by_caller++; break;
+        case 1:  bt->state = BT_STAGED; parsec_list_nolock_push_back(&dev->stalled, &bt->item); dev->nb_stalled++; break;
+        case 2:  parsec_list_nolock_push_back(&dev->cold_q, &bt->item); dev->nb_cold++; break;
         case 3:  bt->state = BT_DMA_IN; parsec_list_nolock_push_back(&dev->waiting_event, &bt->item);
                  if( bt->cold_bytes ) (void)parsec_atomic_fetch_add_int64(&dev->cold_inflight, (int64_t)bt->cold_bytes);
                  break;
@@ -1289,24 +1293,9 @@
     }
     t1 = B200_TSC(); dev->tsc_s[0] += t1 - t0; t0 = t1;
     int started = 0;
-    if( dev->retry_stalled && (dev->nb_settled > 0 || dev->nb_stalled > 0 || dev->nb_cold > 0) ) {
+    if( dev->retry_stalled && (dev->nb_stalled > 0 || dev->nb_cold > 0) ) {
         int ring_full = 0, cut = 0;
         dev->retry_stalled = 0;
-        while( dev->nb_settled > 0 ) {
-            if( started >= 512 ) { cut = 1; break; }
-            b200_task_t *bt = (b200_task_t*)PARSEC_LIST_ITERATOR_FIRST(&dev->settled);
-            parsec_list_item_t *la = PARSEC_LIST_ITERATOR_NEXT(&bt->item);
-            if( la != PARSEC_LIST_ITERATOR_END(&dev->settled) ) { la = PARSEC_LIST_ITERATOR_NEXT(la);
-                if( la != PARSEC_LIST_ITERATOR_END(&dev->settled) ) { B200_PF(la); B200_PF((const char*)la + offsetof(b200_task_t, cmd)); } }
-            parsec_list_nolock_remove(&dev->settled, &bt->item);
-            PARSEC_LIST_ITEM_SINGLETON(&bt->item);
-            if( BT_NEW == bt->state ) bt->state = BT_STAGED;
-            const int rc = b200_push_engine(dev, bt);
-            if( PARSEC_HOOK_RETURN_AGAIN == rc ) { parsec_list_nolock_push_front(&dev->settled, &bt->item); ring_full = 1; break; }
-            if( PARSEC_HOOK_RETURN_DONE != rc ) return -1;
-            dev->nb_settled--;
-            started++;
-        }
         while( !ring_full && !cut && dev->nb_cold > 0 ) {
             if( started >= 512 ) { cut = 1; break; }
             b200_task_t *bt = (b200_task_t*)PARSEC_LIST_ITERATOR_FIRST(&dev->cold_q);
@@ -1365,6 +1354,7 @@
         if( cut ) dev->retry_stalled = 1;
     }
     if( dev->lane_pending > 0 ) { const int n = b200_fire_lane(dev); if( n < 0 ) return -1; moved += n; }
+    dev->n_started += (uint64_t)started;
     if( started && PB2_SUCCESS != pb2_stream_kick(dev->stream) ) return -1;
     t1 = B200_TSC(); dev->tsc_s[1] += t1 - t0; t0 = t1;
     if( !parsec_list_nolock_is_empty(&dev->waiting_event) ) {
@@ -1477,6 +1467,7 @@
                 return -1;
             }
             bt->result = dev->retbuf[i].result;
+            dev->n_engine++;
             if( NULL != dev->trace_ev || (NULL != parsec_b200_trace && '\0' != parsec_b200_trace[0]) ) b200_trace_task(dev, bt, &dev->retbuf[i]);
             if( (PB2_BODY_CHECK_I32 == bt->body || PB2_BODY_CHECK_F32 == bt->body) && (bt->result >> 32) ) dev->st.check_mismatches += bt->result >> 32;
             bt->ticket = -1;
@@ -1498,7 +1489,7 @@
 static inline int b200_start_work(const parsec_device_b200_module_t *dev)
 {
     return dev->inbox_tail != dev->inbox_head ||
-           ((dev->nb_stalled > 0 || dev->nb_settled > 0 || dev->nb_cold > 0) && dev->retry_stalled) ||
+           ((dev->nb_stalled > 0 || dev->nb_cold > 0) && dev->retry_stalled) ||
            !parsec_list_nolock_is_empty((parsec_list_t*)&dev->waiting_event);
 }
 
@@ -1549,7 +1540,6 @@
         dev->inbox_tail - dev->inbox_head < B200_INBOX_SLOTS - 4096  ) {
         b200_lock(&dev->alloc_lock);
         decided = 1;
-        bt->defer_tiles = 1;
         if( PARSEC_HOOK_RETURN_DONE == b200_reserve(dev, bt) ) {
             const int rc = b200_stage_in(dev, bt, 0);
             if( 0 == rc ) { b200_build_cmd(dev, bt); bt->prepared = 2; }
@@ -1558,10 +1548,10 @@
                 bt->prepared = 3;
             } else if( PARSEC_HOOK_RETURN_AGAIN != rc ) dev->fatal = 1;
         }
-        if( 0 == bt->prepared ) bt->defer_tiles = (bt->ntdesc > 0);
     }
     int32_t before = parsec_atomic_fetch_add_int32(&dev->owed, 1);
-    {
+    const int direct = (1 == bt->prepared || 2 == bt->prepared) && b200_submit_direct(dev, bt);
+    if( !direct ) {
         const int64_t idx = parsec_atomic_fetch_add_int64(&dev->inbox_tail, 1);
         while( idx - dev->inbox_head >= B200_INBOX_SLOTS ) { _mm_pause(); }
         parsec_atomic_wmb();
@@ -1586,11 +1576,11 @@
     for(;;) {
         dev->completed_now = 0;
         if( 0 == (++idle_spins & 0x3ffffff) && NULL != getenv("PARSEC_B200_DEBUG") ) {
-            fprintf(stderr, "b200 manager stuck? owed %d inbox %ld stalled %d settled %d starter %d retry %d stream inflight %d executed %lu\n",
-                    dev->owed, (long)(dev->inbox_tail - dev->inbox_head), dev->nb_stalled, dev->nb_settled, dev->starter_active, dev->retry_stalled,
+            fprintf(stderr, "b200 manager stuck? owed %d inbox %ld stalled %d cold %d starter %d retry %d stream inflight %d executed %lu\n",
+                    dev->owed, (long)(dev->inbox_tail - dev->inbox_head), dev->nb_stalled, dev->nb_cold, dev->starter_active, dev->retry_stalled,
                     pb2_stream_inflight(dev->stream), (unsigned long)module->executed_tasks);
         }
-        if( (dev->nb_stalled > 0 || dev->nb_settled > 0 || dev->nb_cold > 0) && ++dev->blocked_spins >= 1024 ) {
+        if( (dev->nb_stalled > 0 || dev->nb_cold > 0) && ++dev->blocked_spins >= 1024 ) {
             dev->blocked_spins = 0; dev->retry_stalled = 1;
         }
         if( b200_start_work(dev) && b200_try_start(dev, es, 0) < 0 ) dev->fatal = 1;
@@ -1726,8 +1716,8 @@
 {
     if( NULL == getenv("PARSEC_B200_PROFILE") ) return;
     uint64_t tot = 0; for( int i = 3; i < 7; i++ ) tot += dev->tsc[i];
-    fprintf(stderr, "b200 starter Mcycles: inbox %.1f start %.1f events %.1f (total %.1f, %lu settled by their caller) | manager Mcycles: poll %.1f finish %.1f idle-poll %.1f schedule %.1f (total %.1f, %lu tasks so far, %lu manager entries)\n",
-            dev->tsc_s[0] * 1e-6, dev->tsc_s[1] * 1e-6, dev->tsc_s[2] * 1e-6, (dev->tsc_s[0] + dev->tsc_s[1] + dev->tsc_s[2]) * 1e-6, (unsigned long)dev->n_settled_by_caller,
+    fprintf(stderr, "b200 starter Mcycles: inbox %.1f start %.1f events %.1f (total %.1f, %lu tasks started by the starter) | manager Mcycles: poll %.1f finish %.1f idle-poll %.1f schedule %.1f (total %.1f, %lu tasks so far, %lu manager entries)\n",
+            dev->tsc_s[0] * 1e-6, dev->tsc_s[1] * 1e-6, dev->tsc_s[2] * 1e-6, (dev->tsc_s[0] + dev->tsc_s[1] + dev->tsc_s[2]) * 1e-6, (unsigned long)dev->n_started,
             dev->tsc[3] * 1e-6, dev->tsc[4] * 1e-6, dev->tsc[5] * 1e-6, dev->tsc[6] * 1e-6,
             tot * 1e-6, (unsigned long)dev->super.super.super.executed_tasks, (unsigned long)dev->st.manager_entries);
     memset(dev->tsc_s, 0, sizeof dev->tsc_s);
@@ -1845,7 +1835,6 @@
     PARSEC_OBJ_CONSTRUCT(&gpu->gpu_mem_owned_lru, parsec_list_t);
     PARSEC_OBJ_CONSTRUCT(&gpu->pending, parsec_fifo_t);
     PARSEC_OBJ_CONSTRUCT(&dev->stalled, parsec_list_t);
-    PARSEC_OBJ_CONSTRUCT(&dev->settled, parsec_list_t);
     PARSEC_OBJ_CONSTRUCT(&dev->waiting_out, parsec_list_t);
     PARSEC_OBJ_CONSTRUCT(&dev->cold_q, parsec_list_t);
     PARSEC_OBJ_CONSTRUCT(&dev->waiting_event, parsec_list_t);
```

Result: no change. 99.37 million (median of 6 runs) (+0.0%).
